# qinzheng93/GeoTransformer

Measured on NVIDIA H100. Metric: point-cloud pairs/sec (3DMatch-shape synth), higher is better.
Workload: dtype f32

## Files before the change

geotransformer_b200/_lib.py:

```python
import ctypes
import os
import threading

import torch

_HERE = os.path.dirname(os.path.abspath(__file__))
LIB_PATH = os.path.join(_HERE, 'libgeob200.so')
_lib = None

c_void_p, c_int64, c_int32, c_float, c_double, c_size_t, c_int = (
    ctypes.c_void_p, ctypes.c_int64, ctypes.c_int32, ctypes.c_float, ctypes.c_double, ctypes.c_size_t, ctypes.c_int)

SIGNATURES = {}


def _sig(name, restype, *argtypes):
    SIGNATURES[name] = (restype, list(argtypes))


P, I64, I32, F, D, SZ = c_void_p, c_int64, c_int32, c_float, c_double, c_size_t
_sig('geob200_last_error', ctypes.c_char_p)
_sig('geob200_launch_count', ctypes.c_uint64)
_sig('geob200_grid_subsample_workspace_bytes', SZ, I64, I64)
_sig('geob200_grid_subsample', c_int, P, I64, P, I64, F, P, P, P, SZ, P)
_sig('geob200_radius_search_workspace_bytes', SZ, I64, I64, I64)
_sig('geob200_radius_search', c_int, P, I64, P, I64, P, P, I64, F, I64, P, P, P, P, SZ, P)

_sig('geob200_neighbor_histogram', c_int, P, I64, I64, I64, I64, P, P)
_sig('geob200_neighbor_histogram_batched', c_int, P, P, P, I64, I64, I64, I64, P, P, P, P)
_sig('geob200_voxel_down_sample_workspace_bytes', SZ, I64, I64)
_sig('geob200_voxel_down_sample', c_int, P, P, I64, P, I64, D, P, P, P, P, SZ, P)
_sig('geob200_estimate_normals_workspace_bytes', SZ, I64, I64)
_sig('geob200_estimate_normals', c_int, P, I64, P, I64, I64, D, P, P, P, P, P, SZ, P)
_sig('geob200_regularize_normals', c_int, P, P, I64, c_int, c_int, P, P)
_sig('geob200_kernel_point_optimize', c_int, P, I64, I64, ctypes.c_uint64, D, P, P, P)
_sig('geob200_kernel_point_instances', c_int, P, I64, P, P, I64, ctypes.c_uint64, P, P)
_sig('geob200_kpconv_workspace_bytes', SZ, I64)
_sig('geob200_kpconv', c_int, P, P, P, P, I64, I64, I64, P, I64, P, P, I64, I64, F, P, P, SZ, P)
_sig('geob200_kpconv_tc_workspace_bytes', SZ, I64, I64, I64)
_sig('geob200_kpconv_tc', c_int, P, P, P, P, I64, I64, I64, P, I64, P, P, I64, I64, F, P, P, SZ, P)
_sig('geob200_set_linear_mode', None, c_int)
_sig('geob200_linear', c_int, P, I64, P, P, P, I64, I64, I64, I64, c_int, P)
_sig('geob200_split_tf32', c_int, P, I64, I64, I64, P, P)
_sig('geob200_linear_batched', c_int, P, I64, I64, P, I64, I64, P, I64, P, I64, I64, I64, I64, I64, I64, c_int, P)
_sig('geob200_group_norm_workspace_bytes', SZ, I64)
_sig('geob200_group_norm', c_int, P, I64, I64, I64, P, P, F, P, c_int, F, P, P, SZ, P)
_sig('geob200_fused_group_norm_workspace_bytes', SZ, I64, I64, I64)
_sig('geob200_linear_group_norm', c_int, P, I64, P, P, I64, I64, I64, I64, P, P, F, P, c_int, F, P, P, P, SZ, P)
_sig('geob200_kpconv_group_norm', c_int, P, P, P, P, I64, I64, I64, P, I64, P, P, I64, I64, F, I64, P, P, F, c_int, F, P, P, P, SZ,
     P, SZ, P)
_sig('geob200_group_norm_batched', c_int, P, I64, I64, I64, P, P, F, P, c_int, F, P, P, SZ, P, I64, P)
_sig('geob200_linear_group_norm_batched', c_int, P, I64, P, P, I64, I64, I64, I64, P, P, F, P, c_int, F, P, P, P, SZ, P, I64, P)
_sig('geob200_maxpool', c_int, P, P, I64, I64, I64, I64, P, P)
_sig('geob200_upsample_concat', c_int, P, P, I64, I64, P, I64, I64, I64, P, P)
_sig('geob200_kpconv_backward_workspace_bytes', SZ, I64, I64, I64, I64, I64)
_sig('geob200_kpconv_backward', c_int, P, P, P, P, I64, I64, I64, P, I64, P, I64, I64, F, P, P, P, P, P, SZ, P)
_sig('geob200_linear_backward_workspace_bytes', SZ, I64, I64, I64, c_int)
_sig('geob200_linear_backward', c_int, P, I64, P, P, I64, I64, I64, P, P, P, P, P, SZ, P)
_sig('geob200_group_norm_backward_batched_workspace_bytes', SZ, I64, I64, I64, I64)
_sig('geob200_group_norm_backward_batched', c_int, P, P, I64, I64, I64, P, F, c_int, F, P, P, P, P, P, P, SZ, P, I64, P)
_sig('geob200_maxpool_backward_batched_workspace_bytes', SZ, I64, I64, I64, I64)
_sig('geob200_maxpool_backward_batched', c_int, P, P, I64, I64, I64, I64, P, I64, P, P, P, P, SZ, P)
_sig('geob200_upsample_concat_backward_workspace_bytes', SZ, I64, I64)
_sig('geob200_upsample_concat_backward', c_int, P, I64, I64, I64, I64, I64, P, P, P, P, SZ, P)
_sig('geob200_point_to_node_partition_batched', c_int, P, P, I64, P, P, I64, P, P, P, P, P, P)
_sig('geob200_gather_rows', c_int, P, I64, I64, P, I64, P, P)
_sig('geob200_knn_partition', c_int, P, I64, P, I64, I64, P, P, P)
_sig('geob200_pairwise_distance', c_int, P, I64, P, I64, I64, c_int, P, P)
_sig('geob200_point_to_node_indices', c_int, P, I64, P, I64, P, P, P)
_sig('geob200_apply_transform', c_int, P, I64, P, P, P)
_sig('geob200_gse_indices_batched', c_int, P, I64, P, F, F, I64, P, P, P)
_sig('geob200_gse_embed_workspace_bytes', SZ, I64, I64)
_sig('geob200_gse_table_bytes', SZ, I64, I64, F, F)
_sig('geob200_gse_table_build', c_int, P, P, P, P, P, I64, I64, F, F, P, SZ, P)
_sig('geob200_gse_embed_table', c_int, P, P, I64, I64, P, SZ, I64, F, F, P, P, P, P, P, P, P)
_sig('geob200_gse_embed_pairs', c_int, P, P, I64, I64, P, P, P, P, P, P, P, P, P, SZ, P)
_sig('geob200_attention_workspace_bytes', SZ, I64, I64, I64)
_sig('geob200_attention', c_int, P, I64, P, I64, P, I64, P, P, P, I64, I64, I64, I64, P, I64, P, SZ, P)
_sig('geob200_set_attention_tma', c_int, c_int)
_sig('geob200_head_bias', c_int, P, I64, P, I64, I64, I64, P, P)
_sig('geob200_add_layernorm', c_int, P, P, P, P, I64, I64, F, P, P)
_sig('geob200_l2_normalize', c_int, P, I64, I64, P, P)
_sig('geob200_add_layernorm_backward_workspace_bytes', SZ, I64, I64)
_sig('geob200_add_layernorm_backward', c_int, P, P, P, I64, I64, F, P, P, P, P, P, SZ, P)
_sig('geob200_l2_normalize_backward', c_int, P, I64, I64, P, P, P)
_sig('geob200_head_project_backward_workspace_bytes', SZ, I64, I64, I64)
_sig('geob200_head_project_backward', c_int, P, I64, P, P, I64, I64, I64, P, P, P, I64, P, P, P, SZ, P)
_sig('geob200_attention_backward_batched_workspace_bytes', SZ, P, I64, I64)
_sig('geob200_attention_backward_batched', c_int, P, P, I64, I64, I64, I64, I64, I64, I64, I64, I64, I64, P, SZ, P)
_sig('geob200_gse_embed_backward_workspace_bytes', SZ, I64, I64)
_sig('geob200_gse_embed_backward', c_int, P, P, I64, I64, I64, P, SZ, I64, F, F, P, P, P, P, P, P, P, P, P, SZ, P)
_sig('geob200_sinkhorn', c_int, P, P, P, P, I64, I64, I64, F, P, P)
_sig('geob200_sinkhorn_backward_workspace_bytes', SZ, I64, I64, I64)
_sig('geob200_sinkhorn_backward', c_int, P, P, P, P, I64, I64, I64, F, P, P, P, P, SZ, P)
_sig('geob200_superpoint_matching_batched_workspace_bytes', SZ, I64, I64, I64)
_sig('geob200_superpoint_matching_batched', c_int, P, P, I64, P, P, I64, P, I64, c_int, P, P, P, P, SZ, P)
_sig('geob200_gather_patches_batched', c_int, P, I64, I64, P, P, P, P, I64, P, P, P, P, P)
_sig('geob200_patch_scores_batched', c_int, P, P, I64, I64, P, P, P, I64, I64, P, P)
_sig('geob200_patch_scores_backward_batched_workspace_bytes', SZ, I64, I64, I64, I64)
_sig('geob200_patch_scores_backward_batched', c_int, P, P, I64, I64, P, P, P, I64, I64, P, P, P, P, SZ, P)
_sig('geob200_lgr_batched_workspace_bytes', SZ, I64, I64, I64, I64)
_sig('geob200_local_global_registration_batched', c_int, P, P, P, P, P, I64, I64, I64, I64, I64, F, c_int, F, I64, I64, P, P, P, P,
     P, P, I64, P, P, P, P, SZ, P)
_sig('geob200_weighted_procrustes', c_int, P, P, P, I64, I64, F, F, P, P)

_sig('geob200_node_correspondences_batched_workspace_bytes', SZ, I64, I64, I64)
_sig('geob200_node_correspondences_batched', c_int, P, P, P, P, P, P, P, P, I64, P, I64, P, F, P, P, P, P, SZ, P)
_sig('geob200_evaluate_counts', c_int, P, P, I64, P, F, P, P, I64, P, P, P, I64, P, F, P, P, P, I64, c_int, F, F, F, P, P)
_sig('geob200_evaluate_batched', c_int, P, P, P, F, P, P, I64, P, P, P, I64, P, F, P, P, I64, P, I64, P, P, c_int, F, F, F, P, I64,
     P)
_sig('geob200_coarse_matching_loss_batched_workspace_bytes', SZ, I64, I64)
_sig('geob200_coarse_matching_loss_batched', c_int, P, P, I64, I64, P, P, P, P, F, F, F, F, F, F, P, I64, P, SZ, P)
_sig('geob200_fine_matching_loss_batched_workspace_bytes', SZ, I64, I64)
_sig('geob200_fine_matching_loss_batched', c_int, P, P, P, P, P, P, I64, I64, I64, P, D, P, P, I64, P, SZ, P)
_sig('geob200_coarse_matching_loss_backward_batched_workspace_bytes', SZ, I64, I64, I64)
_sig('geob200_coarse_matching_loss_backward_batched', c_int, P, P, I64, I64, P, P, P, P, F, F, F, F, F, F, P, I64, P, P, P, P, SZ, P)
_sig('geob200_fine_matching_loss_backward_batched_workspace_bytes', SZ, I64, I64)
_sig('geob200_fine_matching_loss_backward_batched', c_int, P, P, P, P, P, I64, I64, I64, P, D, P, I64, P, P, P, SZ, P)
_sig('geob200_ransac_correspondences_batched_workspace_bytes', SZ, I64, I64)
_sig('geob200_ransac_correspondences_batched', c_int, P, P, I64, I64, P, F, I64, I64, ctypes.c_uint64, I64, P, P, P, P, P, P, P, P, P, P,
     SZ, P)
_sig('geob200_feature_nn_batched_workspace_bytes', SZ, I64, I64, I64)
_sig('geob200_feature_nn_batched', c_int, P, P, I64, I64, I64, I64, P, P, P, P, P, P, P, SZ, P)
_sig('geob200_feature_corr_indices', c_int, P, P, P, P, I64, I64, I32, P, P, P, P, P)
_sig('geob200_ransac_features_batched_workspace_bytes', SZ, I64, I64, I64, I64, I64)
_sig('geob200_ransac_features_batched', c_int, P, P, P, P, I64, I64, I64, I64, P, P, F, I64, I64, I64, ctypes.c_uint64, I64, P, P, P, P, P,
     P, P, P, P, P, P, P, P, P, SZ, P)
_sig('geob200_correspondence_metrics_batched_workspace_bytes', SZ, I64, I64)
_sig('geob200_correspondence_metrics_batched', c_int, P, P, I64, I64, P, P, I64, F, P, I64, P, SZ, P)
_sig('geob200_corr_order_batched', c_int, P, I64, I64, P, I64, P, P)
_sig('geob200_corr_select_batched', c_int, P, P, P, I64, I64, P, P, I64, I64, P, P, P, P, P)
_sig('geob200_sparse_correspondence_eval_batched_workspace_bytes', SZ, I64, I64, I64)
_sig('geob200_sparse_correspondence_eval_batched', c_int, P, P, I64, P, P, I64, P, I64, I64, I64, P, P, SZ, P)
_sig('geob200_registration_error_batched', c_int, P, I64, P, I64, P, P, I64, c_int, D, D, P, P)
_sig('geob200_weighted_procrustes_counts', c_int, P, P, P, I64, I64, P, F, F, P, P)

_sig('geob200_linear_profile_enable', c_int, c_int)
_sig('geob200_set_split_k', c_int, c_int)
_sig('geob200_set_linear_persistent', c_int, c_int)
_sig('geob200_linear_profile_read', I64, I64, P, P)
_sig('geob200_backbone_workspace_bytes', SZ, P, P)
_sig('geob200_backbone_forward_batched', c_int, P, P, P, P, P, P, P, P, P, P, P, P, SZ, P, SZ, P, I64, P, P)
_sig('geob200_cloud_max_count', c_int, P, I64, I64, I64, I64, P, P, P)
_sig('geob200_transformer_batched_workspace_bytes', SZ, I64, P, I64, I64, I64)
_sig('geob200_transformer_forward_batched', c_int, P, I64, I64, I64, P, I64, P, P, P, P, SZ, P)
_sig('geob200_attention_batched_workspace_bytes', SZ, P, I64, I64)
_sig('geob200_attention_batched', c_int, P, I64, I64, I64, I64, I64, I64, I64, P, SZ, P)
_sig('geob200_attention_batched_keeps_probs', c_int, P, I64, I64, I64)
_sig('geob200_superpoint_targets_batched_workspace_bytes', SZ, I64)
_sig('geob200_superpoint_targets_batched', c_int, P, P, P, I64, P, F, I64, ctypes.c_uint64, ctypes.c_uint64, I64, P, P, P, P, SZ, P)
_sig('geob200_nonfinite_check', c_int, P, P, I64, I64, P, P)
_sig('geob200_batch_loss_weights', c_int, P, I64, I64, P, P, P, P, P)
_sig('geob200_kpconv_group_norm_batched', c_int, P, P, P, P, I64, I64, I64, P, I64, P, P, I64, I64, F, I64, P, P, F, c_int, F, P, P, P,
     SZ, P, SZ, P, I64, P)
_sig('geob200_maxpool_batched', c_int, P, P, I64, I64, I64, I64, P, I64, P, P, P)
_sig('geob200_augment_pairs_batched_workspace_bytes', SZ, I64)
_sig('geob200_augment_pairs_batched', c_int, P, P, I64, P, c_int, I64, D, D, D, D, D, ctypes.c_uint64, ctypes.c_uint64, I64, P, P, P, P, P,
     SZ, P)
_sig('geob200_modelnet_pairs_batched_workspace_bytes', SZ, I64)
_sig('geob200_modelnet_pairs_batched', c_int, P, P, I64, I64, D, D, D, D, ctypes.c_uint64, ctypes.c_uint64, I64, P, P, P, P, P, SZ, P)
_sig('geob200_modelnet_benchmark_pairs_batched_workspace_bytes', SZ, I64, I64)
_sig('geob200_modelnet_benchmark_pairs_batched', c_int, P, P, P, I64, I64, D, D, D, D, P, P, P, P, SZ, P)
_sig('geob200_rotated_pairs_batched', c_int, P, c_int, P, P, I64, P, P, P, P, P)
_sig('geob200_modelnet_raw_points_batched_workspace_bytes', SZ, I64)
_sig('geob200_modelnet_raw_points_batched', c_int, P, P, I64, P, P, SZ, P)
_sig('geob200_rpmnet_metrics_batched_workspace_bytes', SZ, I64, I64, I64)
_sig('geob200_rpmnet_metrics_batched', c_int, P, P, P, P, P, P, I64, P, P, P, P, SZ, P)


def lib():
    global _lib
    if _lib is None:
        if not os.path.exists(LIB_PATH):
            raise RuntimeError(
                f'{LIB_PATH} not found: build it with `python -c "import __graft_entry__ as g; g.build()"` '
                '(there is no CPU fallback for the geotransformer_b200 ops)')
        handle = ctypes.CDLL(LIB_PATH)
        for name, (restype, argtypes) in SIGNATURES.items():
            fn = getattr(handle, name)
            fn.restype = restype
            fn.argtypes = argtypes
        _lib = handle
    return _lib


def check(rc, what):
    if rc != 0:
        msg = lib().geob200_last_error().decode(errors='replace')
        raise RuntimeError(f'{what} failed ({rc}): {msg}')


_tls = threading.local()


def stream_ptr():
    p = getattr(_tls, 'stream', None)
    if p is not None:
        return p
    return torch.cuda.current_stream().cuda_stream


class stream_scope:

    def __init__(self, ptr):
        self.ptr = ptr

    def __enter__(self):
        self.prev = getattr(_tls, 'stream', None)
        _tls.stream = self.ptr
        return self

    def __exit__(self, *a):
        _tls.stream = self.prev
        return False


def require_cuda(t, name, dtype=None):
    if not t.is_cuda:
        raise RuntimeError(f'{name} must be a CUDA tensor (geotransformer_b200 has no CPU path)')
    if dtype is not None and t.dtype != dtype:
        raise RuntimeError(f'{name} must be {dtype}, got {t.dtype}')
    if not t.is_contiguous():
        raise RuntimeError(f'{name} must be contiguous')


_WS = {}


def workspace(nbytes, device, tag='default'):
    key = (device.index if device.index is not None else torch.cuda.current_device(), stream_ptr(), tag)
    buf = _WS.get(key)
    if buf is None or buf.numel() < nbytes:
        buf = torch.empty(max(int(nbytes * 1.3), 1 << 20), dtype=torch.uint8, device=device)
        _WS[key] = buf
    return buf


def ptr(t):
    return None if t is None else t.data_ptr()
```

geotransformer_b200/csrc/collate.cu:

```cuda
#include <stdarg.h>
#include <string.h>

#include <mutex>
#include <set>
#include <utility>

#include "common.cuh"
#include "geob200.h"
#include "unordered_map.cuh"

namespace geob200 {

static thread_local char g_err[1024] = "";
static unsigned long long g_launches = 0;
void count_launches(int n) { __atomic_fetch_add(&g_launches, (unsigned long long)n, __ATOMIC_RELAXED); }
void set_error(const char* fmt, ...) {
    va_list ap;
    va_start(ap, fmt);
    vsnprintf(g_err, sizeof(g_err), fmt, ap);
    va_end(ap);
}

int ensure_max_smem(const void* kernel) {
    static std::mutex mu;
    static std::set<std::pair<const void*, int>> done;
    int dev = 0;
    cudaGetDevice(&dev);
    std::lock_guard<std::mutex> lk(mu);
    if (done.count({kernel, dev})) return 0;
    int optin = 0;
    cudaFuncAttributes fa{};
    cudaError_t e = cudaDeviceGetAttribute(&optin, cudaDevAttrMaxSharedMemoryPerBlockOptin, dev);
    if (e == cudaSuccess) e = cudaFuncGetAttributes(&fa, kernel);
    if (e == cudaSuccess) e = cudaFuncSetAttribute(kernel, cudaFuncAttributeMaxDynamicSharedMemorySize, optin - (int)fa.sharedSizeBytes);
    if (e != cudaSuccess) { set_error("ensure_max_smem: %s", cudaGetErrorString(e)); return -1; }
    done.insert({kernel, dev});
    return 0;
}


__global__ void __launch_bounds__(1024) seg_exclusive_scan_kernel(const int* __restrict__ in, int* __restrict__ out,
                                                                  const CloudSeg* __restrict__ segs,
                                                                  int* __restrict__ total) {
    __shared__ int warp_tot[32];
    __shared__ int carry_s;
    const CloudSeg sg = segs[blockIdx.x];
    const int lane = threadIdx.x & 31, warp = threadIdx.x >> 5;
    if (threadIdx.x == 0) carry_s = 0;
    __syncthreads();
    for (int base = 0; base < sg.len; base += 1024) {
        int i = base + threadIdx.x;
        int v = (i < sg.len) ? in[sg.start + i] : 0;
        int x = v;
#pragma unroll
        for (int o = 1; o < 32; o <<= 1) {
            int y = __shfl_up_sync(0xffffffffu, x, o);
            if (lane >= o) x += y;
        }
        if (lane == 31) warp_tot[warp] = x;
        __syncthreads();
        if (warp == 0) {
            int w = warp_tot[lane];
#pragma unroll
            for (int o = 1; o < 32; o <<= 1) {
                int y = __shfl_up_sync(0xffffffffu, w, o);
                if (lane >= o) w += y;
            }
            warp_tot[lane] = w;
        }
        __syncthreads();
        int carry = carry_s;
        int excl = carry + (warp > 0 ? warp_tot[warp - 1] : 0) + (x - v);
        if (i < sg.len) out[sg.start + i] = excl;
        __syncthreads();
        if (threadIdx.x == 1023) carry_s = carry + warp_tot[31];
        __syncthreads();
    }
    if (threadIdx.x == 0 && total != nullptr) total[blockIdx.x] = carry_s;
}


struct GsCloud {
    float ox, oy, oz;
    unsigned long long nx, ny;
};

#define GS_EMPTY 0xFFFFFFFFFFFFFFFFull

__global__ void __launch_bounds__(1024) gs_bounds_kernel(const float* __restrict__ pts, const CloudSeg* __restrict__ segs,
                                                         float voxel, GsCloud* __restrict__ out) {
    const CloudSeg sg = segs[blockIdx.x];
    float mn[3] = {INFINITY, INFINITY, INFINITY}, mx[3] = {-INFINITY, -INFINITY, -INFINITY};
    for (int i = threadIdx.x; i < sg.len; i += blockDim.x) {
        const float* p = pts + 3ll * (sg.start + i);
#pragma unroll
        for (int a = 0; a < 3; ++a) {
            mn[a] = fminf(mn[a], p[a]);
            mx[a] = fmaxf(mx[a], p[a]);
        }
    }
    __shared__ float smn[3][32], smx[3][32];
    const int lane = threadIdx.x & 31, warp = threadIdx.x >> 5;
#pragma unroll
    for (int a = 0; a < 3; ++a) {
#pragma unroll
        for (int o = 16; o > 0; o >>= 1) {
            mn[a] = fminf(mn[a], __shfl_xor_sync(0xffffffffu, mn[a], o));
            mx[a] = fmaxf(mx[a], __shfl_xor_sync(0xffffffffu, mx[a], o));
        }
        if (lane == 0) { smn[a][warp] = mn[a]; smx[a][warp] = mx[a]; }
    }
    __syncthreads();
    if (threadIdx.x == 0) {
        const int nw = blockDim.x >> 5;
        for (int a = 0; a < 3; ++a)
            for (int w = 1; w < nw; ++w) {
                smn[a][0] = fminf(smn[a][0], smn[a][w]);
                smx[a][0] = fmaxf(smx[a][0], smx[a][w]);
            }
        const float inv = (float)(1.0 / (double)voxel);
        GsCloud c;
        c.ox = __fmul_rn(floorf(__fmul_rn(smn[0][0], inv)), voxel);
        c.oy = __fmul_rn(floorf(__fmul_rn(smn[1][0], inv)), voxel);
        c.oz = __fmul_rn(floorf(__fmul_rn(smn[2][0], inv)), voxel);
        c.nx = (unsigned long long)(floorf(__fdiv_rn(__fsub_rn(smx[0][0], c.ox), voxel)) + 1.0f);
        c.ny = (unsigned long long)(floorf(__fdiv_rn(__fsub_rn(smx[1][0], c.oy), voxel)) + 1.0f);
        out[blockIdx.x] = c;
    }
}

__global__ void gs_insert_kernel(const float* __restrict__ pts, const CloudSeg* __restrict__ segs,
                                 const GsCloud* __restrict__ clouds, float voxel,
                                 unsigned long long* __restrict__ tab_key, int* __restrict__ tab_first,
                                 int* __restrict__ pt_slot) {
    const CloudSeg sg = segs[blockIdx.y];
    const int i = blockIdx.x * blockDim.x + threadIdx.x;
    if (i >= sg.len) return;
    const GsCloud c = clouds[blockIdx.y];
    const float* p = pts + 3ll * (sg.start + i);
    unsigned long long ix = (unsigned long long)floorf(__fdiv_rn(__fsub_rn(p[0], c.ox), voxel));
    unsigned long long iy = (unsigned long long)floorf(__fdiv_rn(__fsub_rn(p[1], c.oy), voxel));
    unsigned long long iz = (unsigned long long)floorf(__fdiv_rn(__fsub_rn(p[2], c.oz), voxel));
    unsigned long long key = ix + c.nx * iy + c.nx * c.ny * iz;
    const unsigned tsize = 2u * (unsigned)sg.len;
    const long long tbase = 2ll * sg.start;
    unsigned h = (unsigned)(mix64(key) % tsize);
    while (true) {
        unsigned long long prev = atomicCAS(&tab_key[tbase + h], GS_EMPTY, key);
        if (prev == GS_EMPTY || prev == key) break;
        h = (h + 1 == tsize) ? 0 : h + 1;
    }
    atomicMin(&tab_first[tbase + h], i);
    pt_slot[sg.start + i] = (int)h;
}

__global__ void gs_flag_kernel(const CloudSeg* __restrict__ segs, const int* __restrict__ tab_first,
                               const int* __restrict__ pt_slot, int* __restrict__ flag) {
    const CloudSeg sg = segs[blockIdx.y];
    const int i = blockIdx.x * blockDim.x + threadIdx.x;
    if (i >= sg.len) return;
    flag[sg.start + i] = (tab_first[2ll * sg.start + pt_slot[sg.start + i]] == i) ? 1 : 0;
}

__global__ void gs_offsets_kernel(const int* __restrict__ m, int nb, int* __restrict__ voff, long long* __restrict__ s_lengths) {
    if (threadIdx.x == 0 && blockIdx.x == 0) {
        int acc = 0;
        for (int b = 0; b < nb; ++b) {
            voff[b] = acc;
            acc += m[b];
            s_lengths[b] = m[b];
        }
        voff[nb] = acc;
    }
}

__global__ void gs_voxel_setup_kernel(const float* __restrict__ pts, const CloudSeg* __restrict__ segs,
                                      const GsCloud* __restrict__ clouds, float voxel,
                                      const int* __restrict__ flag, const int* __restrict__ rank,
                                      const int* __restrict__ pt_slot, int* __restrict__ tab_rank,
                                      unsigned long long* __restrict__ vox_key) {
    const CloudSeg sg = segs[blockIdx.y];
    const int i = blockIdx.x * blockDim.x + threadIdx.x;
    if (i >= sg.len) return;
    if (!flag[sg.start + i]) return;
    const GsCloud c = clouds[blockIdx.y];
    const float* p = pts + 3ll * (sg.start + i);
    unsigned long long ix = (unsigned long long)floorf(__fdiv_rn(__fsub_rn(p[0], c.ox), voxel));
    unsigned long long iy = (unsigned long long)floorf(__fdiv_rn(__fsub_rn(p[1], c.oy), voxel));
    unsigned long long iz = (unsigned long long)floorf(__fdiv_rn(__fsub_rn(p[2], c.oz), voxel));
    const int g = rank[sg.start + i];
    tab_rank[2ll * sg.start + pt_slot[sg.start + i]] = g;
    vox_key[sg.start + g] = ix + c.nx * iy + c.nx * c.ny * iz;
}

__global__ void gs_count_kernel(const CloudSeg* __restrict__ segs, const int* __restrict__ tab_rank,
                                const int* __restrict__ pt_slot, int* __restrict__ vox_count) {
    const CloudSeg sg = segs[blockIdx.y];
    const int i = blockIdx.x * blockDim.x + threadIdx.x;
    if (i >= sg.len) return;
    const int g = tab_rank[2ll * sg.start + pt_slot[sg.start + i]];
    atomicAdd(&vox_count[sg.start + g], 1);
}

__global__ void gs_scatter_kernel(const CloudSeg* __restrict__ segs, const int* __restrict__ tab_rank,
                                  const int* __restrict__ pt_slot, const int* __restrict__ vox_off,
                                  int* __restrict__ vox_cursor, int* __restrict__ vox_pts) {
    const CloudSeg sg = segs[blockIdx.y];
    const int i = blockIdx.x * blockDim.x + threadIdx.x;
    if (i >= sg.len) return;
    const int g = tab_rank[2ll * sg.start + pt_slot[sg.start + i]];
    const int pos = atomicAdd(&vox_cursor[sg.start + g], 1);
    vox_pts[sg.start + vox_off[sg.start + g] + pos] = i;
}

__global__ void gs_reduce_kernel(const float* __restrict__ pts, const CloudSeg* __restrict__ segs,
                                 const int* __restrict__ m_per_cloud, const int* __restrict__ vox_off,
                                 const int* __restrict__ vox_count, const int* __restrict__ vox_pts,
                                 float* __restrict__ vox_bary) {
    const CloudSeg sg = segs[blockIdx.y];
    const int g = blockIdx.x * blockDim.x + threadIdx.x;
    if (g >= m_per_cloud[blockIdx.y]) return;
    const int c = vox_count[sg.start + g];
    const int* lst = vox_pts + sg.start + vox_off[sg.start + g];
    float sx = 0.f, sy = 0.f, sz = 0.f;
    int last = -1;
    for (int k = 0; k < c; ++k) {
        int best = 0x7fffffff;
        for (int j = 0; j < c; ++j) {
            int v = lst[j];
            if (v > last && v < best) best = v;
        }
        const float* p = pts + 3ll * (sg.start + best);
        sx = __fadd_rn(sx, p[0]);
        sy = __fadd_rn(sy, p[1]);
        sz = __fadd_rn(sz, p[2]);
        last = best;
    }
    const float w = (float)(1.0 / (double)c);
    float* o = vox_bary + 3ll * (sg.start + g);
    o[0] = __fmul_rn(sx, w);
    o[1] = __fmul_rn(sy, w);
    o[2] = __fmul_rn(sz, w);
}

__global__ void __launch_bounds__(1024) gs_order_kernel(const CloudSeg* __restrict__ segs, const int* __restrict__ m_per_cloud,
                                                        const int* __restrict__ cloud_voff,
                                                        const unsigned long long* __restrict__ vox_key,
                                                        const float* __restrict__ vox_bary,
                                                        int* __restrict__ cur_g, int* __restrict__ nxt_g,
                                                        int* __restrict__ A_g, int* __restrict__ lnk_g,
                                                        int* __restrict__ bucket_scratch,
                                                        float* __restrict__ s_points) {
    const CloudSeg sg = segs[blockIdx.x];
    const int m = m_per_cloud[blockIdx.x];
    int* act = bucket_scratch + (3ll * sg.start + 64ll * blockIdx.x) * 3;
    const long long bcap = 3ll * sg.len + 64;
    const int* order = unordered_map_order(m, vox_key + sg.start, cur_g + sg.start, nxt_g + sg.start, A_g + sg.start,
                                           lnk_g + sg.start, act, act + bcap, act + 2 * bcap);
    float* out = s_points + 3ll * cloud_voff[blockIdx.x];
    for (int q = threadIdx.x; q < m; q += blockDim.x) {
        const float* bsrc = vox_bary + 3ll * (sg.start + order[q]);
        out[3 * q + 0] = bsrc[0];
        out[3 * q + 1] = bsrc[1];
        out[3 * q + 2] = bsrc[2];
    }
}

static int upload_segs(const int64_t* lengths_h, int64_t batch, CloudSeg* d_segs, int64_t* total, int* max_len,
                       cudaStream_t st) {
    CloudSeg tmp[64];
    CloudSeg* h = tmp;
    CloudSeg* heap = nullptr;
    if (batch > 64) { heap = (CloudSeg*)malloc(sizeof(CloudSeg) * batch); h = heap; }
    int64_t acc = 0;
    int mx = 0;
    for (int64_t b = 0; b < batch; ++b) {
        h[b].start = (int)acc;
        h[b].len = (int)lengths_h[b];
        acc += lengths_h[b];
        if ((int)lengths_h[b] > mx) mx = (int)lengths_h[b];
    }
    cudaError_t e = cudaMemcpyAsync(d_segs, h, sizeof(CloudSeg) * batch, cudaMemcpyHostToDevice, st);
    if (heap) { cudaStreamSynchronize(st); free(heap); }
    *total = acc;
    *max_len = mx;
    if (e != cudaSuccess) { set_error("upload_segs: %s", cudaGetErrorString(e)); return -1; }
    return 0;
}


struct RsCloud {
    float ox, oy, oz;
    float cell;
    int cx, cy, cz;
    int cell_base;
};

__global__ void __launch_bounds__(1024) rs_bounds_kernel(const float* __restrict__ pts, const CloudSeg* __restrict__ segs,
                                                         float radius, RsCloud* __restrict__ out, CloudSeg* __restrict__ cell_segs,
                                                         int* __restrict__ max_count) {
    if (blockIdx.x == 0 && threadIdx.x == 0) *max_count = 0;
    const CloudSeg sg = segs[blockIdx.x];
    float mn[3] = {INFINITY, INFINITY, INFINITY}, mx[3] = {-INFINITY, -INFINITY, -INFINITY};
    for (int i = threadIdx.x; i < sg.len; i += blockDim.x) {
        const float* p = pts + 3ll * (sg.start + i);
#pragma unroll
        for (int a = 0; a < 3; ++a) { mn[a] = fminf(mn[a], p[a]); mx[a] = fmaxf(mx[a], p[a]); }
    }
    __shared__ float smn[3][32], smx[3][32];
    const int lane = threadIdx.x & 31, warp = threadIdx.x >> 5;
#pragma unroll
    for (int a = 0; a < 3; ++a) {
#pragma unroll
        for (int o = 16; o > 0; o >>= 1) {
            mn[a] = fminf(mn[a], __shfl_xor_sync(0xffffffffu, mn[a], o));
            mx[a] = fmaxf(mx[a], __shfl_xor_sync(0xffffffffu, mx[a], o));
        }
        if (lane == 0) { smn[a][warp] = mn[a]; smx[a][warp] = mx[a]; }
    }
    __syncthreads();
    if (threadIdx.x == 0) {
        const int nw = blockDim.x >> 5;
        for (int a = 0; a < 3; ++a)
            for (int w = 1; w < nw; ++w) { smn[a][0] = fminf(smn[a][0], smn[a][w]); smx[a][0] = fmaxf(smx[a][0], smx[a][w]); }
        RsCloud c;
        c.ox = smn[0][0]; c.oy = smn[1][0]; c.oz = smn[2][0];
        const long long budget = 2ll * sg.len + 1024;
        float cell = radius * 1.001f;
        long long cx, cy, cz;
        while (true) {
            cx = (long long)floorf((smx[0][0] - c.ox) / cell) + 1;
            cy = (long long)floorf((smx[1][0] - c.oy) / cell) + 1;
            cz = (long long)floorf((smx[2][0] - c.oz) / cell) + 1;
            if (cx <= 1024 && cy <= 1024 && cz <= 1024 && cx * cy * cz <= budget) break;
            cell *= 1.25f;
        }
        c.cell = cell; c.cx = (int)cx; c.cy = (int)cy; c.cz = (int)cz;
        c.cell_base = 2 * sg.start + 1025 * blockIdx.x;
        out[blockIdx.x] = c;
        cell_segs[blockIdx.x].start = c.cell_base;
        cell_segs[blockIdx.x].len = c.cx * c.cy * c.cz + 1;
    }
}

__device__ __forceinline__ int rs_cell_of(const RsCloud& c, float x, float y, float z) {
    int ix = (int)floorf((x - c.ox) / c.cell), iy = (int)floorf((y - c.oy) / c.cell), iz = (int)floorf((z - c.oz) / c.cell);
    ix = min(max(ix, 0), c.cx - 1); iy = min(max(iy, 0), c.cy - 1); iz = min(max(iz, 0), c.cz - 1);
    return (iz * c.cy + iy) * c.cx + ix;
}

__global__ void rs_count_kernel(const float* __restrict__ pts, const CloudSeg* __restrict__ segs,
                                const RsCloud* __restrict__ clouds, int* __restrict__ cell_cnt, int* __restrict__ pt_cell) {
    const CloudSeg sg = segs[blockIdx.y];
    const int i = blockIdx.x * blockDim.x + threadIdx.x;
    if (i >= sg.len) return;
    const RsCloud c = clouds[blockIdx.y];
    const float* p = pts + 3ll * (sg.start + i);
    const int cell = rs_cell_of(c, p[0], p[1], p[2]);
    pt_cell[sg.start + i] = cell;
    atomicAdd(&cell_cnt[c.cell_base + cell], 1);
}

__global__ void rs_scatter_kernel(const float* __restrict__ pts, const CloudSeg* __restrict__ segs,
                                  const RsCloud* __restrict__ clouds, const int* __restrict__ cell_start,
                                  int* __restrict__ cell_cursor, const int* __restrict__ pt_cell,
                                  float4* __restrict__ sorted) {
    const CloudSeg sg = segs[blockIdx.y];
    const int i = blockIdx.x * blockDim.x + threadIdx.x;
    if (i >= sg.len) return;
    const RsCloud c = clouds[blockIdx.y];
    const int cell = pt_cell[sg.start + i];
    const int pos = atomicAdd(&cell_cursor[c.cell_base + cell], 1);
    const float* p = pts + 3ll * (sg.start + i);
    sorted[sg.start + cell_start[c.cell_base + cell] + pos] = make_float4(p[0], p[1], p[2], __int_as_float(i));
}

struct RsSegs {
    int start, len;
};
__global__ void rs_cellsegs_kernel(const RsCloud* __restrict__ clouds, int nb, CloudSeg* __restrict__ cell_segs) {
    int b = blockIdx.x * blockDim.x + threadIdx.x;
    if (b >= nb) return;
    const RsCloud c = clouds[b];
    cell_segs[b].start = c.cell_base;
    cell_segs[b].len = c.cx * c.cy * c.cz + 1;
}

template <int KPL>
__device__ __forceinline__ void warp_bitonic_sort(unsigned long long (&key)[KPL], int lane) {
#pragma unroll
    for (int k = 2; k <= 32 * KPL; k <<= 1) {
#pragma unroll
        for (int j = k >> 1; j > 0; j >>= 1) {
            if (j >= 32) {
                const int rj = j >> 5;
#pragma unroll
                for (int r = 0; r < KPL; ++r) {
                    if ((r & rj) == 0) {
                        const bool up = (((r * 32 + lane) & k) == 0);
                        const unsigned long long a = key[r], b = key[r | rj];
                        const bool swap = (a > b) == up;
                        key[r] = swap ? b : a;
                        key[r | rj] = swap ? a : b;
                    }
                }
            } else {
#pragma unroll
                for (int r = 0; r < KPL; ++r) {
                    const unsigned long long a = key[r];
                    const unsigned long long b = __shfl_xor_sync(0xffffffffu, a, j);
                    const bool up = (((r * 32 + lane) & k) == 0);
                    const bool lower = (lane & j) == 0;
                    const bool take_min = (up == lower);
                    key[r] = take_min ? (a < b ? a : b) : (a > b ? a : b);
                }
            }
        }
    }
}

template <int KPL>
__device__ __forceinline__ void rs_sort_and_store(const unsigned long long* buf, int count, int lane, long long* orow, int width,
                                                  long long start, long long sentinel) {
    unsigned long long key[KPL];
#pragma unroll
    for (int r = 0; r < KPL; ++r) key[r] = (r * 32 + lane < count) ? buf[r * 32 + lane] : 0xFFFFFFFFFFFFFFFFull;
    warp_bitonic_sort<KPL>(key, lane);
#pragma unroll
    for (int r = 0; r < KPL; ++r) {
        const int e = r * 32 + lane;
        if (e < width) orow[e] = (e < count) ? (long long)(unsigned)(key[r] & 0xFFFFFFFFull) + start : sentinel;
    }
    for (int e = 32 * KPL + lane; e < width; e += 32) orow[e] = sentinel;
}

template <int CAP>
__device__ __forceinline__ void rs_query_body(unsigned long long* buf, int lane, int b, int qi,
                                              const float* __restrict__ q_pts, const CloudSeg* __restrict__ q_segs,
                                              const CloudSeg* __restrict__ s_segs, const RsCloud* __restrict__ clouds,
                                              const int* __restrict__ cell_start, const float4* __restrict__ sorted,
                                              float radius, int width, long long sentinel, long long* __restrict__ out,
                                              int* __restrict__ counts, int* __restrict__ max_count,
                                              int* __restrict__ overflow_list, int* __restrict__ overflow_n) {
    const CloudSeg qs = q_segs[b];
    const CloudSeg ss = s_segs[b];
    const RsCloud c = clouds[b];
    const long long row = (long long)qs.start + qi;
    const float qx = q_pts[3 * row], qy = q_pts[3 * row + 1], qz = q_pts[3 * row + 2];
    const float r2 = __fmul_rn(radius, radius);
    const float lim = 2.0e6f;
    const int ix = (int)fminf(fmaxf(floorf((qx - c.ox) / c.cell), -lim), lim);
    const int iy = (int)fminf(fmaxf(floorf((qy - c.oy) / c.cell), -lim), lim);
    const int iz = (int)fminf(fmaxf(floorf((qz - c.oz) / c.cell), -lim), lim);
    int count = 0;
    const int x0 = max(ix - 1, 0), x1 = min(ix + 1, c.cx - 1);
    if (x0 <= x1) {
        for (int dz = -1; dz <= 1; ++dz) {
            const int z = iz + dz;
            if (z < 0 || z >= c.cz) continue;
            for (int dy = -1; dy <= 1; ++dy) {
                const int y = iy + dy;
                if (y < 0 || y >= c.cy) continue;
                const int rowcell = c.cell_base + (z * c.cy + y) * c.cx;
                const int beg = cell_start[rowcell + x0], end = cell_start[rowcell + x1 + 1];
                const int end_pad = beg + ((end - beg + 31) / 32) * 32;
                for (int k = beg + lane; k < end_pad; k += 32) {
                    bool hit = false;
                    unsigned long long kv = 0;
                    if (k < end) {
                        const float4 s = sorted[ss.start + k];
                        const float ex = __fsub_rn(qx, s.x), ey = __fsub_rn(qy, s.y), ez = __fsub_rn(qz, s.z);
                        float d = __fmul_rn(ex, ex);
                        d = __fadd_rn(d, __fmul_rn(ey, ey));
                        d = __fadd_rn(d, __fmul_rn(ez, ez));
                        hit = d < r2;
                        kv = ((unsigned long long)__float_as_uint(d) << 32) | (unsigned)__float_as_int(s.w);
                    }
                    const unsigned msk = __ballot_sync(0xffffffffu, hit);
                    if (hit) {
                        const int pos = count + __popc(msk & ((1u << lane) - 1u));
                        if (pos < CAP) buf[pos] = kv;
                    }
                    count += __popc(msk);
                }
            }
        }
    }
    if (count > CAP) {
        if (lane == 0) {
            if (overflow_list != nullptr) overflow_list[atomicAdd(overflow_n, 1)] = (int)row;
            else atomicExch(max_count, -1 << 30);
        }
        return;
    }
    if (lane == 0) {
        if (counts != nullptr) counts[row] = count;
        atomicMax(max_count, count);
    }
    if (out == nullptr || width <= 0) return;
    __syncwarp();
    long long* orow = out + row * (long long)width;
    if (count <= 32) rs_sort_and_store<1>(buf, count, lane, orow, width, ss.start, sentinel);
    else if (count <= 64) rs_sort_and_store<2>(buf, count, lane, orow, width, ss.start, sentinel);
    else if (count <= 128) rs_sort_and_store<4>(buf, count, lane, orow, width, ss.start, sentinel);
    else if (count <= 256) rs_sort_and_store<8>(buf, count, lane, orow, width, ss.start, sentinel);
    else {
        int n2 = 1;
        while (n2 < count) n2 <<= 1;
        for (int k = count + lane; k < n2; k += 32) buf[k] = 0xFFFFFFFFFFFFFFFFull;
        __syncwarp();
        for (int k = 2; k <= n2; k <<= 1) {
            for (int j = k >> 1; j > 0; j >>= 1) {
                for (int t = lane; t < n2; t += 32) {
                    const int p = t ^ j;
                    if (p > t) {
                        const unsigned long long a = buf[t], bb = buf[p];
                        const bool up = ((t & k) == 0);
                        if ((a > bb) == up) { buf[t] = bb; buf[p] = a; }
                    }
                }
                __syncwarp();
            }
        }
        for (int k = lane; k < width; k += 32)
            orow[k] = (k < count) ? (long long)(unsigned)(buf[k] & 0xFFFFFFFFull) + ss.start : sentinel;
    }
}

template <int CAP>
__global__ void rs_query_kernel(const float* __restrict__ q_pts, const CloudSeg* __restrict__ q_segs,
                                const CloudSeg* __restrict__ s_segs, const RsCloud* __restrict__ clouds,
                                const int* __restrict__ cell_start, const float4* __restrict__ sorted, float radius,
                                int width, long long sentinel, long long* __restrict__ out, int* __restrict__ counts,
                                int* __restrict__ max_count, int* __restrict__ overflow_list, int* __restrict__ overflow_n) {
    extern __shared__ unsigned long long smem_keys[];
    const int warps_per_block = blockDim.x >> 5;
    const int lane = threadIdx.x & 31, warp = threadIdx.x >> 5;
    const int b = blockIdx.y;
    const int qi = blockIdx.x * warps_per_block + warp;
    if (qi >= q_segs[b].len) return;
    rs_query_body<CAP>(smem_keys + (size_t)warp * CAP, lane, b, qi, q_pts, q_segs, s_segs, clouds, cell_start, sorted,
                       radius, width, sentinel, out, counts, max_count, overflow_list, overflow_n);
}

template <int CAP>
__global__ void rs_redo_kernel(const float* __restrict__ q_pts, const CloudSeg* __restrict__ q_segs,
                               const CloudSeg* __restrict__ s_segs, const RsCloud* __restrict__ clouds,
                               const int* __restrict__ cell_start, const float4* __restrict__ sorted, float radius,
                               int width, long long sentinel, long long* __restrict__ out, int* __restrict__ counts,
                               int* __restrict__ max_count, const int* __restrict__ redo_list,
                               const int* __restrict__ redo_n, int nbatch) {
    extern __shared__ unsigned long long smem_keys[];
    const int n = *redo_n;
    for (int w = blockIdx.x; w < n; w += gridDim.x) {
        const int row = redo_list[w];
        int b = 0;
        while (b + 1 < nbatch && row >= q_segs[b + 1].start) ++b;
        rs_query_body<CAP>(smem_keys, threadIdx.x, b, row - q_segs[b].start, q_pts, q_segs, s_segs, clouds, cell_start,
                           sorted, radius, width, sentinel, out, counts, max_count, nullptr, nullptr);
        __syncwarp();
    }
}

__global__ void __launch_bounds__(256) neighbor_histogram_kernel(const long long* __restrict__ nbr, long long rows, int width,
                                                                 long long n_support, int hist_n, int* __restrict__ hist) {
    const long long r = (long long)blockIdx.x * blockDim.x + threadIdx.x;
    if (r >= rows) return;
    int c = 0;
    for (int j = 0; j < width; ++j) c += nbr[r * width + j] < n_support ? 1 : 0;
    if (c < hist_n) atomicAdd(&hist[c], 1);
}

struct HistStages {
    const long long* nbr[GEOB200_MAX_STAGES];
    long long rows[GEOB200_MAX_STAGES];
    int width[GEOB200_MAX_STAGES];
    int cloud_start[GEOB200_MAX_STAGES][2 * GEOB200_HIST_MAX_PAIRS + 1];
};

__global__ void __launch_bounds__(256) neighbor_histogram_batched_kernel(HistStages st, int num_stages, int batch, int hist_n,
                                                                         int* __restrict__ hists) {
    const int s = blockIdx.y;
    const long long r = (long long)blockIdx.x * blockDim.x + threadIdx.x;
    if (r >= st.rows[s]) return;
    const int w = st.width[s];
    const long long* row = st.nbr[s] + r * w;
    int c = 0;
    for (int j = 0; j < w; ++j) c += row[j] < st.rows[s] ? 1 : 0;
    if (c >= hist_n) return;
    int cloud = 0;
    while (cloud + 1 < 2 * batch && r >= st.cloud_start[s][cloud + 1]) ++cloud;
    atomicAdd(&hists[((size_t)(cloud % batch) * num_stages + s) * hist_n + c], 1);
}

__global__ void __launch_bounds__(256) neighbor_histogram_stop_kernel(const int* __restrict__ hists, int num_stages, int batch,
                                                                      int hist_n, long long threshold, int* __restrict__ totals,
                                                                      int* __restrict__ stop) {
    __shared__ long long row_sum[GEOB200_HIST_MAX_PAIRS * GEOB200_MAX_STAGES];
    __shared__ long long base[GEOB200_MAX_STAGES];
    __shared__ int last;
    const int t = threadIdx.x;
    for (int i = t; i < batch * num_stages; i += blockDim.x) {
        long long v = 0;
        for (int h = 0; h < hist_n; ++h) v += hists[(size_t)i * hist_n + h];
        row_sum[i] = v;
    }
    for (int s = t; s < num_stages; s += blockDim.x) {
        long long v = 0;
        for (int h = 0; h < hist_n; ++h) v += totals[(size_t)s * hist_n + h];
        base[s] = v;
    }
    __syncthreads();
    if (t == 0) {
        int found = -1;
        for (int p = 0; p < batch && found < 0; ++p) {
            bool all = true;
            for (int s = 0; s < num_stages; ++s) {
                base[s] += row_sum[p * num_stages + s];
                all = all && base[s] > threshold;
            }
            if (all) found = p;
        }
        *stop = found;
        last = found >= 0 ? found : batch - 1;
    }
    __syncthreads();
    for (int i = t; i < num_stages * hist_n; i += blockDim.x) {
        int v = totals[i];
        for (int p = 0; p <= last; ++p) v += hists[(size_t)p * num_stages * hist_n + i];
        totals[i] = v;
    }
}

}

using namespace geob200;

extern "C" {

const char* geob200_last_error(void) { return g_err; }
uint64_t geob200_launch_count(void) { return g_launches; }

size_t geob200_grid_subsample_workspace_bytes(int64_t n_points, int64_t batch) {
    size_t n = (size_t)n_points, b = (size_t)batch;
    size_t bytes = 0;
    bytes += align_up(sizeof(CloudSeg) * b, 256) + align_up(sizeof(GsCloud) * b, 256);
    bytes += align_up(8 * 2 * n, 256) + align_up(4 * 2 * n, 256) * 2;
    bytes += align_up(4 * n, 256) * 11;
    bytes += align_up(8 * n, 256);
    bytes += align_up(12 * n, 256);
    bytes += align_up(4 * 3 * (3 * n + 64 * b), 256);
    bytes += align_up(4 * (b + 1), 256) * 2;
    return bytes + 4096;
}

int geob200_grid_subsample(const float* points, int64_t n_points, const int64_t* lengths_h, int64_t batch, float voxel,
                           float* s_points, int64_t* s_lengths, void* workspace, size_t workspace_bytes, void* stream) {
    cudaStream_t st = (cudaStream_t)stream;
    GEOB_REQUIRE(batch > 0 && n_points > 0, "grid_subsample: empty input (n=%lld, batch=%lld)", (long long)n_points, (long long)batch);
    GEOB_REQUIRE(voxel > 0.f, "grid_subsample: voxel size must be positive");
    GEOB_REQUIRE(n_points < (1ll << 30), "grid_subsample: too many points");
    for (int64_t b = 0; b < batch; ++b)
        GEOB_REQUIRE(lengths_h[b] > 0, "grid_subsample: cloud %lld is empty (the reference reads points[0])", (long long)b);
    GEOB_REQUIRE(workspace_bytes >= geob200_grid_subsample_workspace_bytes(n_points, batch), "grid_subsample: workspace too small");
    Arena ar(workspace, workspace_bytes);
    const size_t n = (size_t)n_points;
    CloudSeg* segs = ar.take<CloudSeg>(batch);
    GsCloud* clouds = ar.take<GsCloud>(batch);
    unsigned long long* tab_key = ar.take<unsigned long long>(2 * n);
    int* tab_first = ar.take<int>(2 * n);
    int* tab_rank = ar.take<int>(2 * n);
    int* pt_slot = ar.take<int>(n);
    int* flag = ar.take<int>(n);
    int* rank = ar.take<int>(n);
    int* vox_count = ar.take<int>(2 * n);
    int* vox_cursor = vox_count + n;
    int* vox_off = ar.take<int>(n);
    int* vox_pts = ar.take<int>(n);
    int* cur = ar.take<int>(n);
    int* nxt = ar.take<int>(n);
    int* A = ar.take<int>(n);
    int* lnk = ar.take<int>(n);
    unsigned long long* vox_key = ar.take<unsigned long long>(n);
    float* vox_bary = ar.take<float>(3 * n);
    int* bucket_scratch = ar.take<int>(3 * (3 * n + 64 * (size_t)batch));
    int* m_per_cloud = ar.take<int>(batch + 1);
    int* voff = ar.take<int>(batch + 1);
    GEOB_REQUIRE(ar.ok(), "grid_subsample: workspace accounting error");

    int64_t total = 0;
    int max_len = 0;
    if (upload_segs(lengths_h, batch, segs, &total, &max_len, st)) return -1;
    GEOB_REQUIRE(total == n_points, "grid_subsample: sum(lengths)=%lld != n_points=%lld", (long long)total, (long long)n_points);

    GEOB_CHECK_CUDA(cudaMemsetAsync(tab_key, 0xFF, 8 * 2 * n, st));
    GEOB_CHECK_CUDA(cudaMemsetAsync(tab_first, 0x7F, 4 * 2 * n, st));
    GEOB_CHECK_CUDA(cudaMemsetAsync(vox_count, 0, 4 * 2 * n, st));

    const dim3 pgrid((max_len + 255) / 256, (unsigned)batch);
    gs_bounds_kernel<<<(unsigned)batch, 1024, 0, st>>>(points, segs, voxel, clouds);
    gs_insert_kernel<<<pgrid, 256, 0, st>>>(points, segs, clouds, voxel, tab_key, tab_first, pt_slot);
    gs_flag_kernel<<<pgrid, 256, 0, st>>>(segs, tab_first, pt_slot, flag);
    seg_exclusive_scan_kernel<<<(unsigned)batch, 1024, 0, st>>>(flag, rank, segs, m_per_cloud);
    gs_offsets_kernel<<<1, 32, 0, st>>>(m_per_cloud, (int)batch, voff, (long long*)s_lengths);
    gs_voxel_setup_kernel<<<pgrid, 256, 0, st>>>(points, segs, clouds, voxel, flag, rank, pt_slot, tab_rank, vox_key);
    gs_count_kernel<<<pgrid, 256, 0, st>>>(segs, tab_rank, pt_slot, vox_count);
    seg_exclusive_scan_kernel<<<(unsigned)batch, 1024, 0, st>>>(vox_count, vox_off, segs, nullptr);
    gs_scatter_kernel<<<pgrid, 256, 0, st>>>(segs, tab_rank, pt_slot, vox_off, vox_cursor, vox_pts);
    gs_reduce_kernel<<<pgrid, 256, 0, st>>>(points, segs, m_per_cloud, vox_off, vox_count, vox_pts, vox_bary);
    gs_order_kernel<<<(unsigned)batch, 1024, 0, st>>>(segs, m_per_cloud, voff, vox_key, vox_bary, cur, nxt, A, lnk,
                                                     bucket_scratch, s_points);
    GEOB_CHECK_LAUNCH();
    count_launches(11);
    return 0;
}

size_t geob200_radius_search_workspace_bytes(int64_t n_query, int64_t n_support, int64_t batch) {
    size_t ns = (size_t)n_support, nq = (size_t)n_query, b = (size_t)batch;
    size_t cells = 2 * ns + 1025 * b + 64;
    size_t bytes = 0;
    bytes += align_up(sizeof(CloudSeg) * b, 256) * 3 + align_up(sizeof(RsCloud) * b, 256);
    bytes += align_up(4 * cells, 256) * 3 + 1024;
    bytes += align_up(4 * ns, 256);
    bytes += align_up(16 * ns, 256);
    bytes += align_up(4 * nq, 256);
    bytes += 1024;
    return bytes + 4096;
}

int geob200_radius_search(const float* q_points, int64_t n_query, const float* s_points, int64_t n_support,
                          const int64_t* q_lengths_h, const int64_t* s_lengths_h, int64_t batch, float radius,
                          int64_t width, int64_t* out, int32_t* counts, int32_t* max_count, void* workspace,
                          size_t workspace_bytes, void* stream) {
    cudaStream_t st = (cudaStream_t)stream;
    GEOB_REQUIRE(batch > 0 && n_query > 0 && n_support > 0, "radius_search: empty input");
    GEOB_REQUIRE(radius > 0.f, "radius_search: radius must be positive");
    GEOB_REQUIRE(max_count != nullptr, "radius_search: max_count output is required");
    GEOB_REQUIRE(n_query < (1ll << 30) && n_support < (1ll << 30), "radius_search: too many points");
    GEOB_REQUIRE(workspace_bytes >= geob200_radius_search_workspace_bytes(n_query, n_support, batch), "radius_search: workspace too small");
    for (int64_t b = 0; b < batch; ++b)
        GEOB_REQUIRE(q_lengths_h[b] >= 0 && s_lengths_h[b] > 0, "radius_search: cloud %lld has no support points", (long long)b);
    Arena ar(workspace, workspace_bytes);
    const size_t ns = (size_t)n_support;
    const size_t cells = 2 * ns + 1025 * (size_t)batch + 64;
    CloudSeg* q_segs = ar.take<CloudSeg>(batch);
    CloudSeg* s_segs = ar.take<CloudSeg>(batch);
    CloudSeg* cell_segs = ar.take<CloudSeg>(batch);
    RsCloud* clouds = ar.take<RsCloud>(batch);
    int* zero_block = ar.take<int>(2 * cells + 64);
    int* cell_cnt = zero_block;
    int* cell_cursor = zero_block + cells;
    int* overflow_n = zero_block + 2 * cells;
    int* cell_start = ar.take<int>(cells);
    int* pt_cell = ar.take<int>(ns);
    float4* sorted = ar.take<float4>(ns);
    int* overflow_list = ar.take<int>((size_t)n_query);
    GEOB_REQUIRE(ar.ok(), "radius_search: workspace accounting error");

    int64_t tq = 0, ts = 0;
    int max_q = 0, max_s = 0;
    if (upload_segs(q_lengths_h, batch, q_segs, &tq, &max_q, st)) return -1;
    if (upload_segs(s_lengths_h, batch, s_segs, &ts, &max_s, st)) return -1;
    GEOB_REQUIRE(tq == n_query && ts == n_support, "radius_search: lengths do not sum to the row counts");

    GEOB_CHECK_CUDA(cudaMemsetAsync(zero_block, 0, 4 * (2 * cells + 64), st));

    const dim3 sgrid((max_s + 255) / 256, (unsigned)batch);
    rs_bounds_kernel<<<(unsigned)batch, 1024, 0, st>>>(s_points, s_segs, radius, clouds, cell_segs, max_count);
    rs_count_kernel<<<sgrid, 256, 0, st>>>(s_points, s_segs, clouds, cell_cnt, pt_cell);
    seg_exclusive_scan_kernel<<<(unsigned)batch, 1024, 0, st>>>(cell_cnt, cell_start, cell_segs, nullptr);
    rs_scatter_kernel<<<sgrid, 256, 0, st>>>(s_points, s_segs, clouds, cell_start, cell_cursor, pt_cell, sorted);
    if (max_q > 0) {
        constexpr int CAP = 256, WARPS = 4;
        const dim3 qgrid((max_q + WARPS - 1) / WARPS, (unsigned)batch);
        rs_query_kernel<CAP><<<qgrid, WARPS * 32, WARPS * CAP * 8, st>>>(
            q_points, q_segs, s_segs, clouds, cell_start, sorted, radius, (int)width, (long long)n_support,
            (long long*)out, counts, max_count, overflow_list, overflow_n);
        constexpr int CAP2 = 16384;
        if (ensure_max_smem((const void*)rs_redo_kernel<CAP2>)) return -1;
        rs_redo_kernel<CAP2><<<num_sms(), 32, CAP2 * 8, st>>>(
            q_points, q_segs, s_segs, clouds, cell_start, sorted, radius, (int)width, (long long)n_support,
            (long long*)out, counts, max_count, overflow_list, overflow_n, (int)batch);
        count_launches(2);
    }
    GEOB_CHECK_LAUNCH();
    count_launches(4);
    return 0;
}

int geob200_neighbor_histogram(const int64_t* neighbors, int64_t n_rows, int64_t width, int64_t n_support, int64_t hist_n,
                               int32_t* hist, void* stream) {
    GEOB_REQUIRE(n_rows > 0 && width > 0 && hist_n > 0, "neighbor_histogram: empty input");
    neighbor_histogram_kernel<<<(unsigned)((n_rows + 255) / 256), 256, 0, (cudaStream_t)stream>>>(
        (const long long*)neighbors, (long long)n_rows, (int)width, (long long)n_support, (int)hist_n, hist);
    GEOB_CHECK_LAUNCH();
    count_launches(1);
    return 0;
}

int geob200_neighbor_histogram_batched(const int64_t* const* neighbors, const int64_t* widths, const int64_t* cloud_rows,
                                       int64_t num_stages, int64_t batch, int64_t hist_n, int64_t sample_threshold, int32_t* hists,
                                       int32_t* totals, int32_t* stop, void* stream) {
    GEOB_REQUIRE(num_stages >= 1 && num_stages <= GEOB200_MAX_STAGES, "neighbor_histogram_batched: num_stages must be in 1..%d",
                 GEOB200_MAX_STAGES);
    GEOB_REQUIRE(batch >= 1 && batch <= GEOB200_HIST_MAX_PAIRS, "neighbor_histogram_batched: batch must be in 1..%d",
                 GEOB200_HIST_MAX_PAIRS);
    GEOB_REQUIRE(hist_n >= 1 && hist_n <= (1 << 20), "neighbor_histogram_batched: hist_n must be in 1..2^20");
    GEOB_REQUIRE(neighbors != nullptr && widths != nullptr && cloud_rows != nullptr && hists != nullptr && totals != nullptr &&
                 stop != nullptr, "neighbor_histogram_batched: null pointer");
    HistStages st;
    long long max_rows = 0;
    for (int s = 0; s < (int)num_stages; ++s) {
        GEOB_REQUIRE(neighbors[s] != nullptr && widths[s] >= 1 && widths[s] <= (1 << 20),
                     "neighbor_histogram_batched: stage %d has no table or a bad width", s);
        long long row = 0;
        for (int c = 0; c < 2 * (int)batch; ++c) {
            GEOB_REQUIRE(cloud_rows[s * 2 * batch + c] >= 1, "neighbor_histogram_batched: stage %d cloud %d is empty", s, c);
            st.cloud_start[s][c] = (int)row;
            row += cloud_rows[s * 2 * batch + c];
            GEOB_REQUIRE(row < (1LL << 31), "neighbor_histogram_batched: stage %d has 2^31 rows or more", s);
        }
        st.cloud_start[s][2 * batch] = (int)row;
        st.nbr[s] = (const long long*)neighbors[s];
        st.rows[s] = row;
        st.width[s] = (int)widths[s];
        max_rows = row > max_rows ? row : max_rows;
    }
    cudaStream_t cs = (cudaStream_t)stream;
    GEOB_CHECK_CUDA(cudaMemsetAsync(hists, 0, sizeof(int32_t) * (size_t)batch * num_stages * hist_n, cs));
    neighbor_histogram_batched_kernel<<<dim3((unsigned)((max_rows + 255) / 256), (unsigned)num_stages), 256, 0, cs>>>(
        st, (int)num_stages, (int)batch, (int)hist_n, hists);
    neighbor_histogram_stop_kernel<<<1, 256, 0, cs>>>(hists, (int)num_stages, (int)batch, (int)hist_n, (long long)sample_threshold,
                                                      totals, stop);
    GEOB_CHECK_LAUNCH();
    count_launches(2);
    return 0;
}

}
```

geotransformer_b200/ext.py:

```python

import torch

from . import _lib as L


def _prep(points, lengths, pname, lname):
    if points.dtype != torch.float32:
        raise RuntimeError(f'{pname} must be a float tensor')
    if lengths.dtype != torch.int64:
        raise RuntimeError(f'{lname} must be an long tensor')
    if not points.is_contiguous():
        raise RuntimeError(f'{pname} must be contiguous')
    if not lengths.is_contiguous():
        raise RuntimeError(f'{lname} must be contiguous')
    was_cpu = not points.is_cuda
    if was_cpu:
        points = points.cuda()
    lengths_h = lengths.cpu() if lengths.is_cuda else lengths
    return points, lengths_h, was_cpu


def grid_subsampling(points, lengths, voxel_size):
    dev_lengths = lengths.device
    points, lengths_h, was_cpu = _prep(points, lengths, 'points', 'lengths')
    n, b = points.shape[0], lengths_h.shape[0]
    lib = L.lib()
    ws_bytes = lib.geob200_grid_subsample_workspace_bytes(n, b)
    ws = L.workspace(ws_bytes, points.device)
    s_points = torch.empty((n, 3), dtype=torch.float32, device=points.device)
    s_lengths = torch.empty((b,), dtype=torch.int64, device=points.device)
    L.check(lib.geob200_grid_subsample(points.data_ptr(), n, lengths_h.data_ptr(), b, float(voxel_size),
                                       s_points.data_ptr(), s_lengths.data_ptr(), ws.data_ptr(), ws.numel(),
                                       L.stream_ptr()), 'grid_subsampling')
    s_lengths_h = s_lengths.cpu()
    total = int(s_lengths_h.sum())
    s_points = s_points[:total].clone()
    if was_cpu:
        return [s_points.cpu(), s_lengths_h]
    return [s_points, s_lengths if dev_lengths.type == 'cuda' else s_lengths_h]


def _radius_call(q_points, s_points, ql_h, sl_h, radius, width, out, counts, max_count):
    lib = L.lib()
    nq, ns, b = q_points.shape[0], s_points.shape[0], ql_h.shape[0]
    ws_bytes = lib.geob200_radius_search_workspace_bytes(nq, ns, b)
    ws = L.workspace(ws_bytes, q_points.device)
    L.check(lib.geob200_radius_search(q_points.data_ptr(), nq, s_points.data_ptr(), ns, ql_h.data_ptr(),
                                      sl_h.data_ptr(), b, float(radius), int(width), L.ptr(out), L.ptr(counts),
                                      max_count.data_ptr(), ws.data_ptr(), ws.numel(), L.stream_ptr()),
            'radius_neighbors')


def radius_neighbors(q_points, s_points, q_lengths, s_lengths, radius, neighbor_limit=0):
    q_points, ql_h, was_cpu = _prep(q_points, q_lengths, 'q_points', 'q_lengths')
    s_points, sl_h, _ = _prep(s_points, s_lengths, 's_points', 's_lengths')
    nq = q_points.shape[0]
    dev = q_points.device
    max_count = torch.zeros((1,), dtype=torch.int32, device=dev)
    if neighbor_limit > 0:
        out = torch.empty((nq, neighbor_limit), dtype=torch.int64, device=dev)
        _radius_call(q_points, s_points, ql_h, sl_h, radius, neighbor_limit, out, None, max_count)
        mc = int(max_count.item())
        if mc < 0:
            raise RuntimeError('radius_neighbors: more than 16384 neighbours for one query')
        if mc < neighbor_limit:
            out = out[:, :mc].contiguous()
    else:
        _radius_call(q_points, s_points, ql_h, sl_h, radius, 0, None, None, max_count)
        mc = int(max_count.item())
        if mc < 0:
            raise RuntimeError('radius_neighbors: more than 16384 neighbours for one query')
        out = torch.empty((nq, mc), dtype=torch.int64, device=dev)
        if mc > 0:
            _radius_call(q_points, s_points, ql_h, sl_h, radius, mc, out, None, max_count)
    return out.cpu() if was_cpu else out


def radius_neighbors_deferred(q_points, s_points, q_lengths, s_lengths, radius, neighbor_limit):
    q_points, ql_h, _ = _prep(q_points, q_lengths, 'q_points', 'q_lengths')
    s_points, sl_h, _ = _prep(s_points, s_lengths, 's_points', 's_lengths')
    dev = q_points.device
    max_count = torch.empty((1,), dtype=torch.int32, device=dev)
    out = torch.empty((q_points.shape[0], neighbor_limit), dtype=torch.int64, device=dev)
    _radius_call(q_points, s_points, ql_h, sl_h, radius, neighbor_limit, out, None, max_count)
    return out, max_count
```

geotransformer_b200/modules/ops/__init__.py:

```python
import torch

from ... import ext as _ext
from ... import functional as GF


def grid_subsample(points, lengths, voxel_size):
    s_points, s_lengths = _ext.grid_subsampling(points, lengths, voxel_size)
    return s_points, s_lengths


def radius_search(q_points, s_points, q_lengths, s_lengths, radius, neighbor_limit):
    return _ext.radius_neighbors(q_points, s_points, q_lengths, s_lengths, radius, neighbor_limit=max(int(neighbor_limit), 0))


def radius_search_deferred(q_points, s_points, q_lengths, s_lengths, radius, neighbor_limit):
    return _ext.radius_neighbors_deferred(q_points, s_points, q_lengths, s_lengths, radius, int(neighbor_limit))


def point_to_node_partition(points, nodes, point_limit, return_count=False):
    return GF.point_to_node_partition(points, nodes, point_limit, return_count)


def knn_partition(points, nodes, k, return_distance=False):
    return GF.knn_partition(points, nodes, k, return_distance)


def get_point_to_node_indices(points, nodes, return_counts=False):
    return GF.point_to_node_indices(points, nodes, return_counts)


def ball_query_partition(points, nodes, radius, point_limit, return_count=False):
    node_knn_distances, node_knn_indices = GF.knn_partition(points, nodes, point_limit, return_distance=True)
    node_knn_masks = torch.lt(node_knn_distances, radius)
    node_knn_indices = torch.where(node_knn_masks, node_knn_indices, torch.full_like(node_knn_indices, points.shape[0]))
    if return_count:
        return node_knn_indices, node_knn_masks, node_knn_masks.sum(1)
    return node_knn_indices, node_knn_masks


def pairwise_distance(x, y, normalized=False, channel_first=False):
    return GF.pairwise_distance(x, y, normalized, channel_first)


def index_select(data, index, dim):
    if dim == 0 and data.is_cuda and data.dtype == torch.float32 and data.ndim == 2 and data.is_contiguous():
        return GF.gather_rows(data, index.contiguous())
    out = data.index_select(dim, index.reshape(-1))
    if index.ndim > 1:
        out = out.view(*data.shape[:dim], *index.shape, *data.shape[dim:][1:])
    return out


def apply_transform(points, transform):
    if transform.ndim == 2:
        return GF.apply_transform(points, transform.contiguous())
    return torch.stack([GF.apply_transform(p, t.contiguous()) for p, t in zip(points, transform)])
```

geotransformer_b200/utils/data.py:

```python
import ctypes

import numpy as np
import torch

from ..modules.ops import grid_subsample, radius_search_deferred


def precompute_data_stack_mode(points, lengths, num_stages, voxel_size, radius, neighbor_limits):
    assert num_stages == len(neighbor_limits)
    points_list, lengths_list, lengths_host = [], [], []
    for i in range(num_stages):
        if i > 0:
            points, lengths = grid_subsample(points, lengths_host[-1], voxel_size=voxel_size)
        lengths_h = lengths.cpu() if lengths.is_cuda else lengths
        points_list.append(points)
        lengths_host.append(lengths_h)
        lengths_list.append(lengths_h.to(points.device))
        voxel_size *= 2

    pending = []
    for i in range(num_stages):
        cur_points, cur_lengths = points_list[i], lengths_host[i]
        pending.append(('n', radius_search_deferred(cur_points, cur_points, cur_lengths, cur_lengths, radius, neighbor_limits[i])))
        if i < num_stages - 1:
            sub_points, sub_lengths = points_list[i + 1], lengths_host[i + 1]
            pending.append(('s', radius_search_deferred(sub_points, cur_points, sub_lengths, cur_lengths, radius, neighbor_limits[i])))
            pending.append(('u', radius_search_deferred(cur_points, sub_points, cur_lengths, sub_lengths, radius * 2,
                                                        neighbor_limits[i + 1])))
        radius *= 2
    counts = torch.stack([p[1][1] for p in pending]).cpu().flatten().tolist()
    neighbors_list, subsampling_list, upsampling_list = [], [], []
    for (kind, (table, _)), mc in zip(pending, counts):
        if mc < 0:
            raise RuntimeError('radius_search: more than 16384 neighbours for one query')
        if mc < table.shape[1]:
            table = table[:, :mc].contiguous()
        {'n': neighbors_list, 's': subsampling_list, 'u': upsampling_list}[kind].append(table)
    return {'points': points_list, 'lengths': lengths_list, 'lengths_host': [l.tolist() for l in lengths_host],
            'neighbors': neighbors_list, 'subsampling': subsampling_list, 'upsampling': upsampling_list}


def _stack_to_device(tensors, device):
    if all(t.is_cuda for t in tensors):
        return tensors[0] if len(tensors) == 1 else torch.cat(tensors, dim=0)
    total = sum(int(t.shape[0]) for t in tensors)
    out = torch.empty((total,) + tuple(tensors[0].shape[1:]), dtype=tensors[0].dtype, device=device)
    row = 0
    for t in tensors:
        out[row:row + t.shape[0]].copy_(t, non_blocking=True)
        row += t.shape[0]
    return out


def registration_collate_fn_stack_mode(data_dicts, num_stages, voxel_size, search_radius, neighbor_limits,
                                       precompute_data=True, device='cuda'):
    batch_size = len(data_dicts)
    collated = {}
    for d in data_dicts:
        for key, value in d.items():
            if isinstance(value, np.ndarray):
                value = torch.from_numpy(value)
            collated.setdefault(key, []).append(value)
    feats_list = collated.pop('ref_feats') + collated.pop('src_feats')
    points_list = collated.pop('ref_points') + collated.pop('src_points')
    lengths = torch.LongTensor([p.shape[0] for p in points_list])
    if batch_size == 1:
        for key, value in collated.items():
            collated[key] = value[0]
    def _dev(v):
        if isinstance(v, torch.Tensor):
            return v.to(device, non_blocking=True)
        if isinstance(v, list) and v and all(isinstance(x, torch.Tensor) for x in v):
            return [x.to(device, non_blocking=True) for x in v]
        return v
    collated = {k: _dev(v) for k, v in collated.items()}
    points, feats = _stack_to_device(points_list, device), _stack_to_device(feats_list, device)
    collated['features'] = feats
    if precompute_data:
        collated.update(precompute_data_stack_mode(points, lengths, num_stages, voxel_size, search_radius, neighbor_limits))
    else:
        collated['points'] = points
        collated['lengths'] = lengths
    collated['batch_size'] = batch_size
    return collated


def calibrate_neighbors_stack_mode(dataset, collate_fn, num_stages, voxel_size, search_radius, keep_ratio=0.8, sample_threshold=2000):
    from .. import _lib as L
    hist_n = int(np.ceil(4 / 3 * np.pi * (search_radius / voxel_size + 1) ** 3))
    max_neighbor_limits = [hist_n] * num_stages
    hists = None
    lib = L.lib()
    for i in range(len(dataset)):
        data_dict = collate_fn([dataset[i]], num_stages, voxel_size, search_radius, max_neighbor_limits, precompute_data=True)
        if hists is None:
            hists = torch.zeros((num_stages, hist_n), dtype=torch.int32, device=data_dict['neighbors'][0].device)
        for s, neighbors in enumerate(data_dict['neighbors']):
            L.check(lib.geob200_neighbor_histogram(neighbors.data_ptr(), neighbors.shape[0], neighbors.shape[1], neighbors.shape[0],
                                                   hist_n, hists[s].data_ptr(), L.stream_ptr()), 'neighbor_histogram')
        if int(hists.sum(dim=1).min().item()) > sample_threshold:
            break
    neighbor_hists = hists.cpu().numpy()
    cum_sum = np.cumsum(neighbor_hists.T, axis=0)
    neighbor_limits = np.sum(cum_sum < (keep_ratio * cum_sum[hist_n - 1, :]), axis=0)
    return neighbor_limits


CALIBRATION_ITERATION = (1 << 64) - 1
HIST_MAX_PAIRS = 32


def calibrate_neighbors_augmented(pairs, cfg, seed, keep_ratio=0.8, sample_threshold=2000, chunk=16, device=None):
    from .. import _lib as L
    from ..augment import augment_stacked
    if not 1 <= chunk <= HIST_MAX_PAIRS:
        raise ValueError(f'chunk must be in 1..{HIST_MAX_PAIRS}')
    device = torch.device('cuda', torch.cuda.current_device()) if device is None else torch.device(device)
    b = cfg.backbone
    S, voxel_size, radius = b.num_stages, b.init_voxel_size, b.init_radius
    hist_n = int(np.ceil(4 / 3 * np.pi * (radius / voxel_size + 1) ** 3))
    totals = torch.zeros((S, hist_n), dtype=torch.int32, device=device)
    hists = torch.empty((chunk, S, hist_n), dtype=torch.int32, device=device)
    stop = torch.empty((1,), dtype=torch.int32, device=device)
    lib = L.lib()
    n, used = len(pairs), len(pairs)
    with torch.cuda.device(device):
        for base in range(0, n, chunk):
            group = [pairs[i] for i in range(base, min(n, base + chunk))]
            B = len(group)
            points, lengths, _, _, _ = augment_stacked(group, cfg, seed, CALIBRATION_ITERATION, device, pair_base=base)
            data = precompute_data_stack_mode(points, torch.LongTensor(lengths), S, voxel_size, radius, [hist_n] * S)
            tables = data['neighbors']
            ptrs = (ctypes.c_void_p * S)(*[t.data_ptr() for t in tables])
            widths = np.array([t.shape[1] for t in tables], dtype=np.int64)
            rows = np.array(data['lengths_host'], dtype=np.int64).reshape(S, 2 * B)
            L.check(lib.geob200_neighbor_histogram_batched(ptrs, widths.ctypes.data, rows.ctypes.data, S, B, hist_n, sample_threshold,
                                                           hists.data_ptr(), totals.data_ptr(), stop.data_ptr(), L.stream_ptr()),
                    'neighbor_histogram_batched')
            p = int(stop.item())
            if p >= 0:
                used = base + p + 1
                break
    cum_sum = np.cumsum(totals.cpu().numpy().T, axis=0)
    return np.sum(cum_sum < (keep_ratio * cum_sum[hist_n - 1, :]), axis=0), used
```

include/geob200.h:

```cpp
#ifndef GEOB200_H
#define GEOB200_H

#include <stddef.h>
#include <stdint.h>

#ifdef __cplusplus
extern "C" {
#endif

const char* geob200_last_error(void);
uint64_t geob200_launch_count(void);


size_t geob200_grid_subsample_workspace_bytes(int64_t n_points, int64_t batch);
int geob200_grid_subsample(const float* points, int64_t n_points, const int64_t* lengths_h, int64_t batch, float voxel,
                           float* s_points, int64_t* s_lengths, void* workspace, size_t workspace_bytes, void* stream);

size_t geob200_radius_search_workspace_bytes(int64_t n_query, int64_t n_support, int64_t batch);
int geob200_radius_search(const float* q_points, int64_t n_query, const float* s_points, int64_t n_support,
                          const int64_t* q_lengths_h, const int64_t* s_lengths_h, int64_t batch, float radius,
                          int64_t width, int64_t* out, int32_t* counts, int32_t* max_count, void* workspace,
                          size_t workspace_bytes, void* stream);

int geob200_neighbor_histogram(const int64_t* neighbors, int64_t n_rows, int64_t width, int64_t n_support, int64_t hist_n,
                               int32_t* hist, void* stream);

#define GEOB200_HIST_MAX_PAIRS 32
int geob200_neighbor_histogram_batched(const int64_t* const* neighbors, const int64_t* widths, const int64_t* cloud_rows,
                                       int64_t num_stages, int64_t batch, int64_t hist_n, int64_t sample_threshold, int32_t* hists,
                                       int32_t* totals, int32_t* stop, void* stream);


#define GEOB200_VOXEL_MAX_CLOUDS 64
#define GEOB200_VOXEL_NONFINITE 1
#define GEOB200_VOXEL_TOO_SMALL 2
#define GEOB200_VOXEL_AXIS_LIMIT 3
size_t geob200_voxel_down_sample_workspace_bytes(int64_t n_points, int64_t batch);
int geob200_voxel_down_sample(const double* points, const double* normals, int64_t n_points, const int64_t* lengths_h, int64_t batch,
                              double voxel, double* out_points, double* out_normals, int64_t* out_lengths, void* workspace,
                              size_t workspace_bytes, void* stream);


#define GEOB200_NORMALS_MAX_CLOUDS 64
#define GEOB200_NORMALS_MAX_KNN 64
#define GEOB200_NORMALS_NONFINITE 1
size_t geob200_estimate_normals_workspace_bytes(int64_t n_points, int64_t batch);
int geob200_estimate_normals(const double* points, int64_t n_points, const int64_t* lengths_h, int64_t batch, int64_t knn, double radius,
                             double* out_normals, int32_t* out_neighbors, double* out_covariance, int64_t* out_status, void* workspace,
                             size_t workspace_bytes, void* stream);
int geob200_regularize_normals(const void* points, const void* normals, int64_t n, int fp64, int positive, double* out, void* stream);


#define GEOB200_KP_MAX_POINTS 30
int geob200_kernel_point_optimize(const double* init, int64_t num_kernels, int64_t num_points, uint64_t seed, double ratio,
                                  double* points, int32_t* info, void* stream);

int geob200_kernel_point_instances(const double* disposition, int64_t num_points, const double* radii, const int64_t* layer_ids,
                                   int64_t num_layers, uint64_t seed, float* out, void* stream);


size_t geob200_kpconv_workspace_bytes(int64_t n_support);
int geob200_kpconv(const float* s_feats, const float* q_points, const float* s_points, const int64_t* neighbors,
                   int64_t n_query, int64_t n_support, int64_t n_neighbors, const float* kernel_points, int64_t n_kernel,
                   const float* weights, const float* bias, int64_t c_in, int64_t c_out, float sigma, float* out,
                   void* workspace, size_t workspace_bytes, void* stream);

size_t geob200_kpconv_tc_workspace_bytes(int64_t n_query, int64_t n_support, int64_t c_in);
int geob200_kpconv_tc(const float* s_feats, const float* q_points, const float* s_points, const int64_t* neighbors, int64_t n_query,
                      int64_t n_support, int64_t n_neighbors, const float* kernel_points, int64_t n_kernel, const float* weights_t,
                      const float* bias, int64_t c_in, int64_t c_out, float sigma, float* out, void* workspace, size_t workspace_bytes,
                      void* stream);

int geob200_split_tf32(const float* w, int64_t ld, int64_t n, int64_t k, float* out, void* stream);

void geob200_set_linear_mode(int mode);
int geob200_linear(const float* x, int64_t ldx, const float* weight, const float* bias, float* y, int64_t ldy, int64_t m,
                   int64_t n, int64_t k, int relu, void* stream);
int geob200_linear_batched(const float* x, int64_t ldx, int64_t stride_x, const float* weight, int64_t ldw, int64_t stride_w,
                           const float* bias, int64_t stride_b, float* y, int64_t ldy, int64_t stride_y, int64_t m, int64_t n,
                           int64_t k, int64_t batch, int relu, void* stream);

size_t geob200_group_norm_workspace_bytes(int64_t groups);
int geob200_group_norm(const float* x, int64_t n_rows, int64_t channels, int64_t groups, const float* gamma,
                       const float* beta, float eps, const float* residual, int leaky, float slope, float* y,
                       void* workspace, size_t workspace_bytes, void* stream);

size_t geob200_fused_group_norm_workspace_bytes(int64_t n_rows, int64_t channels, int64_t groups);
int geob200_linear_group_norm(const float* x, int64_t ldx, const float* weight, const float* bias, int64_t m, int64_t n, int64_t k,
                              int64_t groups, const float* gamma, const float* beta, float eps, const float* residual, int leaky,
                              float slope, float* pre_norm, float* y, void* workspace, size_t workspace_bytes, void* stream);
int geob200_kpconv_group_norm(const float* s_feats, const float* q_points, const float* s_points, const int64_t* neighbors,
                              int64_t n_query, int64_t n_support, int64_t n_neighbors, const float* kernel_points, int64_t n_kernel,
                              const float* weights_t, const float* bias, int64_t c_in, int64_t c_out, float sigma, int64_t groups,
                              const float* gamma, const float* beta, float eps, int leaky, float slope, float* pre_norm, float* y,
                              void* gn_workspace, size_t gn_workspace_bytes, void* workspace, size_t workspace_bytes, void* stream);

int geob200_group_norm_batched(const float* x, int64_t n_rows, int64_t channels, int64_t groups, const float* gamma, const float* beta,
                               float eps, const float* residual, int leaky, float slope, float* y, void* workspace, size_t workspace_bytes,
                               void* stream, int64_t n_pairs, const int64_t* cloud_rows_h);
int geob200_linear_group_norm_batched(const float* x, int64_t ldx, const float* weight, const float* bias, int64_t m, int64_t n, int64_t k,
                                      int64_t groups, const float* gamma, const float* beta, float eps, const float* residual, int leaky,
                                      float slope, float* pre_norm, float* y, void* workspace, size_t workspace_bytes, void* stream,
                                      int64_t n_pairs, const int64_t* cloud_rows_h);
int geob200_kpconv_group_norm_batched(const float* s_feats, const float* q_points, const float* s_points, const int64_t* neighbors,
                                      int64_t n_query, int64_t n_support, int64_t n_neighbors, const float* kernel_points, int64_t n_kernel,
                                      const float* weights_t, const float* bias, int64_t c_in, int64_t c_out, float sigma, int64_t groups,
                                      const float* gamma, const float* beta, float eps, int leaky, float slope, float* pre_norm, float* y,
                                      void* gn_workspace, size_t gn_workspace_bytes, void* workspace, size_t workspace_bytes, void* stream,
                                      int64_t n_pairs, const int64_t* cloud_rows_h);

int geob200_maxpool(const float* x, const int64_t* neighbors, int64_t n_query, int64_t n_support, int64_t n_neighbors,
                    int64_t channels, float* y, void* stream);
int geob200_maxpool_batched(const float* x, const int64_t* neighbors, int64_t n_query, int64_t n_support, int64_t n_neighbors,
                            int64_t channels, const int32_t* cloud_max, int64_t n_pairs, const int64_t* cloud_rows_h, float* y,
                            void* stream);

int geob200_cloud_max_count(const int64_t* neighbors, int64_t n_query, int64_t n_support, int64_t n_neighbors, int64_t n_pairs,
                            const int64_t* cloud_rows_h, int32_t* cloud_max, void* stream);

int geob200_upsample_concat(const float* x, const int64_t* up_indices, int64_t up_stride, int64_t n_support,
                            const float* skip, int64_t n_query, int64_t c1, int64_t c2, float* y, void* stream);


size_t geob200_kpconv_backward_workspace_bytes(int64_t n_query, int64_t n_support, int64_t n_neighbors, int64_t c_in, int64_t c_out);
int geob200_kpconv_backward(const float* s_feats, const float* q_points, const float* s_points, const int64_t* neighbors, int64_t n_query,
                            int64_t n_support, int64_t n_neighbors, const float* kernel_points, int64_t n_kernel, const float* weights,
                            int64_t c_in, int64_t c_out, float sigma, const float* grad_out, float* grad_feats, float* grad_weights,
                            float* grad_bias, void* workspace, size_t workspace_bytes, void* stream);

size_t geob200_linear_backward_workspace_bytes(int64_t m, int64_t n, int64_t k, int relu);
int geob200_linear_backward(const float* x, int64_t ldx, const float* weight_t, const float* relu_y, int64_t m, int64_t n, int64_t k,
                            const float* grad_y, float* grad_x, float* grad_weight, float* grad_bias, void* workspace, size_t workspace_bytes,
                            void* stream);

size_t geob200_group_norm_backward_batched_workspace_bytes(int64_t n_rows, int64_t channels, int64_t groups, int64_t n_pairs);
int geob200_group_norm_backward_batched(const float* x, const float* y, int64_t n_rows, int64_t channels, int64_t groups, const float* gamma,
                                        float eps, int leaky, float slope, const float* grad_y, float* grad_x, float* grad_gamma,
                                        float* grad_beta, float* grad_residual, void* workspace, size_t workspace_bytes, void* stream,
                                        int64_t n_pairs, const int64_t* cloud_rows_h);

size_t geob200_maxpool_backward_batched_workspace_bytes(int64_t n_query, int64_t n_support, int64_t n_neighbors, int64_t channels);
int geob200_maxpool_backward_batched(const float* x, const int64_t* neighbors, int64_t n_query, int64_t n_support, int64_t n_neighbors,
                                     int64_t channels, const int32_t* cloud_max, int64_t n_pairs, const int64_t* cloud_rows_h,
                                     const float* grad_y, float* grad_x, void* workspace, size_t workspace_bytes, void* stream);

size_t geob200_upsample_concat_backward_workspace_bytes(int64_t n_query, int64_t n_support);
int geob200_upsample_concat_backward(const int64_t* up_indices, int64_t up_stride, int64_t n_query, int64_t n_support, int64_t c1, int64_t c2,
                                     const float* grad_y, float* grad_x, float* grad_skip, void* workspace, size_t workspace_bytes,
                                     void* stream);


int geob200_point_to_node_partition_batched(const float* points, const float* nodes, int64_t n_clouds, const int64_t* cloud_points,
                                            const int64_t* cloud_nodes, int64_t point_limit, int64_t* point_to_node, uint8_t* node_masks,
                                            int32_t* node_sizes, int64_t* node_knn_indices, uint8_t* node_knn_masks, void* stream);

int geob200_knn_partition(const float* points, int64_t n_points, const float* nodes, int64_t n_nodes, int64_t k,
                          int64_t* knn_indices, float* knn_sq_distances, void* stream);
int geob200_pairwise_distance(const float* x, int64_t n, const float* y, int64_t m, int64_t channels, int normalized, float* out,
                              void* stream);
int geob200_point_to_node_indices(const float* points, int64_t n_points, const float* nodes, int64_t n_nodes, int64_t* indices,
                                  int32_t* node_sizes, void* stream);
int geob200_apply_transform(const float* points, int64_t n_points, const float* transform, float* out, void* stream);

int geob200_gather_rows(const float* table, int64_t n_rows, int64_t channels, const int64_t* indices, int64_t n_indices,
                        float* out, void* stream);


int geob200_gse_indices_batched(const float* points, int64_t n_clouds, const int64_t* cloud_rows_h, float sigma_d, float factor_a,
                                int64_t angle_k, float* d_indices, float* a_indices, void* stream);

size_t geob200_gse_embed_workspace_bytes(int64_t n, int64_t channels);
int geob200_gse_embed_pairs(const float* d_indices, const float* a_indices, int64_t n_rows, int64_t channels, const float* div_term,
                            const float* wd_t, const float* wa_t, const float* wd, const float* wa, const float* bd, const float* ba,
                            float* embeddings, void* workspace, size_t workspace_bytes, void* stream);

size_t geob200_gse_table_bytes(int64_t channels, int64_t inv_step, float d_max, float a_max);
int geob200_gse_table_build(const float* div_term, const float* wd_t, const float* wa_t, const float* bd, const float* ba,
                            int64_t channels, int64_t inv_step, float d_max, float a_max, void* table, size_t table_bytes,
                            void* stream);
int geob200_gse_embed_table(const float* d_indices, const float* a_indices, int64_t n_rows, int64_t channels, const void* table,
                            size_t table_bytes, int64_t inv_step, float d_max, float a_max, const float* div_term, const float* wd,
                            const float* wa, const float* bd, const float* ba, float* embeddings, void* stream);

size_t geob200_attention_workspace_bytes(int64_t n_query, int64_t n_key, int64_t heads);
int geob200_attention(const float* q, int64_t ldq, const float* k, int64_t ldk, const float* v, int64_t ldv, const float* qp,
                      const float* qb, const float* embed, int64_t n_query, int64_t n_key, int64_t channels, int64_t heads,
                      float* out, int64_t ldo, void* workspace, size_t workspace_bytes, void* stream);
#define GEOB200_ATT_MAX_ITEMS 32
typedef struct { const float* q; const float* k; const float* v; const float* qp; const float* qb; const float* embed; float* out;
                 int64_t n_query, n_key; } geob200_att_item_t;
size_t geob200_attention_batched_workspace_bytes(const geob200_att_item_t* items_h, int64_t n_items, int64_t heads);
int geob200_attention_batched(const geob200_att_item_t* items_h, int64_t n_items, int64_t ldq, int64_t ldk, int64_t ldv, int64_t ldo,
                              int64_t channels, int64_t heads, void* workspace, size_t workspace_bytes, void* stream);
int geob200_attention_batched_keeps_probs(const geob200_att_item_t* items_h, int64_t n_items, int64_t channels, int64_t heads);
int geob200_set_attention_tma(int on);
int geob200_head_bias(const float* q, int64_t ldq, const float* bias_p, int64_t n, int64_t channels, int64_t heads, float* qb,
                      void* stream);
int geob200_add_layernorm(const float* a, const float* b, const float* gamma, const float* beta, int64_t n, int64_t channels,
                          float eps, float* y, void* stream);
int geob200_l2_normalize(const float* x, int64_t n, int64_t channels, float* y, void* stream);


size_t geob200_add_layernorm_backward_workspace_bytes(int64_t n, int64_t channels);
int geob200_add_layernorm_backward(const float* a, const float* b, const float* gamma, int64_t n, int64_t channels, float eps,
                                   const float* grad_y, float* grad_x, float* grad_gamma, float* grad_beta, void* workspace,
                                   size_t workspace_bytes, void* stream);
int geob200_l2_normalize_backward(const float* x, int64_t n, int64_t channels, const float* grad_y, float* grad_x, void* stream);
size_t geob200_head_project_backward_workspace_bytes(int64_t n, int64_t channels, int64_t heads);
int geob200_head_project_backward(const float* q, int64_t ldq, const float* wp, const float* bp, int64_t n, int64_t channels, int64_t heads,
                                  const float* grad_qp, const float* grad_qb, float* grad_q, int64_t ldgq, float* grad_wp, float* grad_bp,
                                  void* workspace, size_t workspace_bytes, void* stream);
typedef struct { const float* probs; const float* grad_out; float* grad_q; float* grad_k; float* grad_v; float* grad_qp; float* grad_qb;
                 float* grad_embed; } geob200_att_grad_item_t;
size_t geob200_attention_backward_batched_workspace_bytes(const geob200_att_item_t* items_h, int64_t n_items, int64_t heads);
int geob200_attention_backward_batched(const geob200_att_item_t* items_h, const geob200_att_grad_item_t* grads_h, int64_t n_items,
                                       int64_t ldq, int64_t ldk, int64_t ldv, int64_t ldo, int64_t ldgq, int64_t ldgk, int64_t ldgv,
                                       int64_t channels, int64_t heads, void* workspace, size_t workspace_bytes, void* stream);
size_t geob200_gse_embed_backward_workspace_bytes(int64_t n_rows, int64_t channels);
int geob200_gse_embed_backward(const float* d_indices, const float* a_indices, int64_t n_rows, int64_t angle_k, int64_t channels,
                               const void* table, size_t table_bytes, int64_t inv_step, float d_max, float a_max, const float* div_term,
                               const float* wa, const float* ba, const float* grad_embed, float* grad_wd, float* grad_bd, float* grad_wa,
                               float* grad_ba, void* workspace, size_t workspace_bytes, void* stream);


size_t geob200_superpoint_matching_batched_workspace_bytes(int64_t n_rows, int64_t n_products, int64_t n_pairs);
int geob200_superpoint_matching_batched(const float* ref_feats, const float* src_feats, int64_t channels, const uint8_t* ref_masks,
                                        const uint8_t* src_masks, int64_t n_pairs, const int64_t* cloud_nodes, int64_t num_correspondences,
                                        int dual, int64_t* corr_indices, float* corr_scores, int32_t* num_out, void* workspace,
                                        size_t workspace_bytes, void* stream);

int geob200_gather_patches_batched(const int64_t* corr_indices, int64_t n_corr, int64_t n_clouds, const int64_t* cloud_nodes,
                                   const int64_t* cloud_points, const int64_t* node_knn_indices, const uint8_t* node_knn_masks, int64_t k,
                                   const float* points, int64_t* out_indices, uint8_t* out_masks, float* out_points, void* stream);

int geob200_patch_scores_batched(const float* ref_feats, const float* src_feats, int64_t channels, int64_t n_pairs, const int64_t* cloud_points,
                                 const int64_t* ref_knn_indices, const int64_t* src_knn_indices, int64_t n_patches, int64_t k,
                                 float* scores, void* stream);

size_t geob200_patch_scores_backward_batched_workspace_bytes(int64_t n_rows, int64_t n_patches_total, int64_t k, int64_t channels);
int geob200_patch_scores_backward_batched(const float* ref_feats, const float* src_feats, int64_t channels, int64_t n_pairs,
                                          const int64_t* cloud_points, const int64_t* ref_knn_indices, const int64_t* src_knn_indices,
                                          int64_t n_patches, int64_t k, const float* grad_scores, float* grad_ref_feats,
                                          float* grad_src_feats, void* workspace, size_t workspace_bytes, void* stream);

int geob200_sinkhorn(const float* scores, const uint8_t* row_masks, const uint8_t* col_masks, const float* alpha,
                     int64_t n_patches, int64_t k, int64_t num_iterations, float inf, float* out, void* stream);

size_t geob200_sinkhorn_backward_workspace_bytes(int64_t n_patches, int64_t k, int64_t num_iterations);
int geob200_sinkhorn_backward(const float* scores, const uint8_t* row_masks, const uint8_t* col_masks, const float* alpha, int64_t n_patches,
                              int64_t k, int64_t num_iterations, float inf, const float* grad_out, float* grad_scores, float* grad_alpha,
                              void* workspace, size_t workspace_bytes, void* stream);


size_t geob200_lgr_batched_workspace_bytes(int64_t n_pairs, int64_t n_patches, int64_t k, int64_t topk);
int geob200_local_global_registration_batched(const float* ref_knn_points, const float* src_knn_points, const uint8_t* ref_knn_masks,
                                              const uint8_t* src_knn_masks, const float* log_scores, int64_t n_pairs, int64_t n_patches,
                                              int64_t k, int64_t score_ld, int64_t topk, float acceptance_radius, int mutual,
                                              float confidence_threshold, int64_t correspondence_threshold, int64_t num_refinement_steps,
                                              float* ref_corr_points, float* src_corr_points, float* corr_scores, int32_t* corr_patch,
                                              int32_t* num_corr, float* estimated_transform, int64_t transform_ld, float* patch_transforms,
                                              int32_t* patch_inliers, int32_t* best_patch, void* workspace, size_t workspace_bytes,
                                              void* stream);

int geob200_weighted_procrustes(const float* src_points, const float* ref_points, const float* weights, int64_t batch,
                                int64_t n, float weight_thresh, float eps, float* transforms, void* stream);

size_t geob200_node_correspondences_batched_workspace_bytes(int64_t n_rows, int64_t n_products, int64_t k);
int geob200_node_correspondences_batched(const float* ref_nodes, const float* src_nodes, const float* ref_knn_points,
                                         const float* src_knn_points, const uint8_t* ref_masks, const uint8_t* src_masks,
                                         const uint8_t* ref_knn_masks, const uint8_t* src_knn_masks, int64_t n_pairs, const int64_t* cloud_nodes,
                                         int64_t k, const float* transforms, float pos_radius, int64_t* corr_indices, float* corr_overlaps,
                                         int32_t* count, void* workspace, size_t workspace_bytes, void* stream);

int geob200_evaluate_counts(const int64_t* gt_node_corr_indices, const float* gt_node_corr_overlaps, int64_t n_gt, const int32_t* n_gt_dev,
                            float acceptance_overlap, const int64_t* ref_node_corr_indices, const int64_t* src_node_corr_indices,
                            int64_t n_node_corr, const int32_t* n_node_corr_dev, const float* ref_corr_points, const float* src_corr_points,
                            int64_t n_corr, const int32_t* n_corr_dev, float acceptance_radius, const float* gt_transform,
                            const float* est_transform, const float* src_points, int64_t n_src_points, int mode, float rmse_threshold,
                            float rre_threshold, float rte_threshold, float* metrics, void* stream);
int geob200_evaluate_batched(const int64_t* gt_node_corr_indices, const float* gt_node_corr_overlaps, const int32_t* n_gt_dev,
                             float acceptance_overlap, const int64_t* ref_node_corr_indices, const int64_t* src_node_corr_indices,
                             int64_t n_node_corr, const int32_t* n_node_corr_dev, const float* ref_corr_points, const float* src_corr_points,
                             int64_t n_corr, const int32_t* n_corr_dev, float acceptance_radius, const float* gt_transforms,
                             const float* est_transforms, int64_t transform_ld, const float* points, int64_t n_pairs, const int64_t* cloud_nodes,
                             const int64_t* cloud_points, int mode, float rmse_threshold, float rre_threshold, float rte_threshold,
                             float* metrics, int64_t metrics_ld, void* stream);

size_t geob200_coarse_matching_loss_batched_workspace_bytes(int64_t n_rows, int64_t n_products);
int geob200_coarse_matching_loss_batched(const float* ref_feats, const float* src_feats, int64_t channels, int64_t n_pairs,
                                         const int64_t* cloud_nodes, const int64_t* gt_node_corr_indices, const float* gt_node_corr_overlaps,
                                         const int32_t* gt_count, float positive_margin, float negative_margin, float positive_optimal,
                                         float negative_optimal, float log_scale, float positive_overlap, float* out, int64_t out_ld,
                                         void* workspace, size_t workspace_bytes, void* stream);
size_t geob200_fine_matching_loss_batched_workspace_bytes(int64_t n_pairs, int64_t n_patches);
int geob200_fine_matching_loss_batched(const float* ref_knn_points, const float* src_knn_points, const uint8_t* ref_knn_masks,
                                       const uint8_t* src_knn_masks, const float* matching_scores, const float* transforms, int64_t n_pairs,
                                       int64_t n_patches, int64_t k, const int32_t* patch_count, double positive_radius,
                                       const float* loss_weights, float* out, int64_t out_ld, void* workspace, size_t workspace_bytes,
                                       void* stream);

size_t geob200_coarse_matching_loss_backward_batched_workspace_bytes(int64_t n_rows, int64_t n_products, int64_t n_pairs);
int geob200_coarse_matching_loss_backward_batched(const float* ref_feats, const float* src_feats, int64_t channels, int64_t n_pairs,
                                                  const int64_t* cloud_nodes, const int64_t* gt_node_corr_indices,
                                                  const float* gt_node_corr_overlaps, const int32_t* gt_count, float positive_margin,
                                                  float negative_margin, float positive_optimal, float negative_optimal, float log_scale,
                                                  float positive_overlap, const float* grad_rows, int64_t grad_ld, const float* loss_weights,
                                                  float* grad_ref_feats, float* grad_src_feats, void* workspace, size_t workspace_bytes,
                                                  void* stream);
size_t geob200_fine_matching_loss_backward_batched_workspace_bytes(int64_t n_pairs, int64_t n_patches);
int geob200_fine_matching_loss_backward_batched(const float* ref_knn_points, const float* src_knn_points, const uint8_t* ref_knn_masks,
                                                const uint8_t* src_knn_masks, const float* transforms, int64_t n_pairs, int64_t n_patches,
                                                int64_t k, const int32_t* patch_count, double positive_radius, const float* grad_rows,
                                                int64_t grad_ld, const float* loss_weights, float* grad_scores, void* workspace,
                                                size_t workspace_bytes, void* stream);

size_t geob200_ransac_correspondences_batched_workspace_bytes(int64_t n_pairs, int64_t num_iterations);
int geob200_ransac_correspondences_batched(const float* ref_corr_points, const float* src_corr_points, int64_t n_pairs, int64_t capacity,
                                           const int32_t* num_corr, float distance_threshold, int64_t ransac_n, int64_t num_iterations,
                                           uint64_t seed, int64_t pair_base, float* transforms, float* fitness, float* inlier_rmse,
                                           int32_t* inlier_count,
                                           int32_t* best_iteration, float* hyp_transforms, int32_t* hyp_inliers, float* hyp_rmse,
                                           int32_t* hyp_samples, void* workspace, size_t workspace_bytes, void* stream);

size_t geob200_correspondence_metrics_batched_workspace_bytes(int64_t n_pairs, int64_t capacity);
int geob200_correspondence_metrics_batched(const float* ref_corr_points, const float* src_corr_points, int64_t n_pairs, int64_t capacity,
                                           const int32_t* num_corr, const float* transforms, int64_t transform_ld, float positive_radius,
                                           float* out, int64_t out_ld, void* workspace, size_t workspace_bytes, void* stream);

size_t geob200_feature_nn_batched_workspace_bytes(int64_t n_pairs, int64_t cap_query, int64_t cap_support);
int geob200_feature_nn_batched(const float* query, const float* support, int64_t n_pairs, int64_t cap_query, int64_t cap_support,
                               int64_t channels, const int32_t* n_query, const int32_t* n_support, int64_t* query_index,
                               double* query_dist, int64_t* support_index, double* support_dist, void* workspace, size_t workspace_bytes,
                               void* stream);
int geob200_feature_corr_indices(const int64_t* ref_nn, const double* ref_dist, const int64_t* src_nn, const double* src_dist,
                                 int64_t n_ref, int64_t n_src, int32_t mode, int64_t* ref_corr, int64_t* src_corr, float* feat_dist,
                                 int32_t* count, void* stream);
size_t geob200_ransac_features_batched_workspace_bytes(int64_t n_pairs, int64_t cap_src, int64_t cap_ref, int64_t num_iterations,
                                                       int64_t val_iterations);
int geob200_ransac_features_batched(const float* src_points, const float* ref_points, const float* src_feats, const float* ref_feats,
                                    int64_t n_pairs, int64_t cap_src, int64_t cap_ref, int64_t channels, const int32_t* n_src,
                                    const int32_t* n_ref, float distance_threshold, int64_t ransac_n, int64_t num_iterations,
                                    int64_t val_iterations, uint64_t seed, int64_t pair_base, float* transforms, float* fitness,
                                    float* inlier_rmse, int32_t* inlier_count, int32_t* best_iteration, int32_t* num_validated,
                                    int64_t* rec_matches, int32_t* rec_samples, int32_t* rec_pass, int32_t* rec_val_ids,
                                    float* rec_transforms, int32_t* rec_inliers, float* rec_rmse, void* workspace, size_t workspace_bytes,
                                    void* stream);

int geob200_corr_order_batched(const float* scores, int64_t n_pairs, int64_t capacity, const int32_t* num_corr, int64_t kmax, int32_t* order,
                               void* stream);
int geob200_corr_select_batched(const float* ref_corr_points, const float* src_corr_points, const float* corr_scores, int64_t n_pairs,
                                int64_t capacity, const int32_t* num_corr, const int32_t* order, int64_t kmax, int64_t k,
                                float* ref_out, float* src_out, float* scores_out, int32_t* count_out, void* stream);
size_t geob200_sparse_correspondence_eval_batched_workspace_bytes(int64_t n_pairs, int64_t m_cap, int64_t n_cap);
int geob200_sparse_correspondence_eval_batched(const int64_t* ref_node_corr_indices, const int64_t* src_node_corr_indices, int64_t pred_cap,
                                               const int32_t* pred_count, const int64_t* gt_node_corr_indices, int64_t gt_cap,
                                               const int32_t* gt_count, int64_t n_pairs, int64_t m_cap, int64_t n_cap, double* out,
                                               void* workspace, size_t workspace_bytes, void* stream);
int geob200_registration_error_batched(const float* gt_transforms, int64_t gt_ld, const float* est_transforms, int64_t est_ld,
                                       const float* covariances, const int32_t* has_covariance, int64_t n_pairs, int mode,
                                       double threshold0, double threshold1, double* out, void* stream);
int geob200_weighted_procrustes_counts(const float* src_points, const float* ref_points, const float* weights, int64_t batch,
                                       int64_t capacity, const int32_t* counts, float weight_thresh, float eps, float* transforms,
                                       void* stream);

int geob200_linear_profile_enable(int on);
int geob200_set_split_k(int on);
int geob200_set_linear_persistent(int on);
int64_t geob200_linear_profile_read(int64_t capacity, int64_t* shapes, float* ms);

#define GEOB200_MAX_STAGES 6
typedef struct { const float* weight; const float* bias; int64_t c_in, c_out; const float* weight_img; } geob200_linear_t;
typedef struct { const float* gamma; const float* beta; } geob200_norm_t;
typedef struct { const float* weights; const float* weights_t; const float* bias; const float* kernel_points;
                 int64_t c_in, c_out; float sigma; const float* weights_img; } geob200_kpconv_t;
typedef struct {
    int32_t has_unary1, has_shortcut, strided, reserved;
    int64_t c_in;
    geob200_linear_t unary1; geob200_norm_t norm1;
    geob200_kpconv_t conv;   geob200_norm_t norm_conv;
    geob200_linear_t unary2; geob200_norm_t norm2;
    geob200_linear_t shortcut; geob200_norm_t norm_sc;
} geob200_resblock_t;
typedef struct {
    int32_t num_stages, finest_decoder, groups, init_dim;
    geob200_kpconv_t conv1; geob200_norm_t norm1;
    geob200_resblock_t blocks[1 + 3 * (GEOB200_MAX_STAGES - 1)];
    geob200_linear_t decoders[GEOB200_MAX_STAGES];
    geob200_norm_t decoder_norms[GEOB200_MAX_STAGES];
} geob200_backbone_t;
size_t geob200_backbone_workspace_bytes(const geob200_backbone_t* net, const int64_t* level_rows);
int geob200_backbone_forward_batched(const geob200_backbone_t* net, const float* feats, const float* const* points,
                                     const int64_t* level_rows, const int64_t* const* neighbors, const int64_t* neighbor_width,
                                     const int64_t* const* subsampling, const int64_t* subsampling_width,
                                     const int64_t* const* upsampling, const int64_t* upsampling_width, float* const* out_feats,
                                     void* gn_workspace, size_t gn_workspace_bytes, void* workspace, size_t workspace_bytes, void* stream,
                                     int64_t n_pairs, const int64_t* const* cloud_rows_h, const int32_t* const* sub_cloud_max);

typedef struct {
    int32_t is_self, reserved;
    const float* w_qkv; const float* b_qkv; const float* w_q; const float* b_q; const float* w_kv; const float* b_kv;
    const float* wp_t; const float* bp;
    geob200_linear_t att_linear; geob200_norm_t att_norm;
    geob200_linear_t expand; geob200_linear_t squeeze; geob200_norm_t out_norm;
    const float* w_qkv_img; const float* w_q_img; const float* w_kv_img;
} geob200_tlayer_t;
size_t geob200_transformer_batched_workspace_bytes(int64_t n_pairs, const int64_t* cloud_rows_h, int64_t channels, int64_t heads,
                                                   int64_t num_layers);
int geob200_transformer_forward_batched(const geob200_tlayer_t* layers, int64_t num_layers, int64_t channels, int64_t heads,
                                        const float* x, int64_t n_pairs, const int64_t* cloud_rows_h, const float* const* embeddings_h,
                                        float* out, void* workspace, size_t workspace_bytes, void* stream);

size_t geob200_superpoint_targets_batched_workspace_bytes(int64_t n_gt_rows);
int geob200_superpoint_targets_batched(const int64_t* gt_indices, const float* gt_overlaps, const int32_t* gt_count, int64_t n_pairs,
                                       const int64_t* cloud_nodes, float overlap_threshold, int64_t num_targets, uint64_t seed,
                                       uint64_t iteration, int64_t pair_base, int64_t* corr_indices, float* corr_scores, int32_t* num_out,
                                       void* workspace, size_t workspace_bytes, void* stream);

int geob200_nonfinite_check(const float* const* ptrs, const int64_t* numels, int64_t n_tensors, int64_t max_numel, float* found_inf,
                            void* stream);

int geob200_batch_loss_weights(const float* loss_rows, int64_t ld_rows, int64_t n_pairs, float* weights, float* mean_row, float* n_valid,
                               float* found_inf, void* stream);

#define GEOB200_AUGMENT_3DMATCH 0
#define GEOB200_AUGMENT_KITTI 1
#define GEOB200_AUGMENT_TAG_BASE 0xA6000000u

size_t geob200_augment_pairs_batched_workspace_bytes(int64_t n_rows);
int geob200_augment_pairs_batched(const float* points, const int64_t* lengths_h, int64_t n_pairs, const float* transforms, int mode,
                                  int64_t point_limit, double noise, double rotation_factor, double min_scale, double max_scale,
                                  double shift, uint64_t seed, uint64_t iteration, int64_t pair_base, float* out_points, int32_t* origin,
                                  float* out_transforms, double* record, void* workspace, size_t workspace_bytes, void* stream);

size_t geob200_modelnet_pairs_batched_workspace_bytes(int64_t n_rows);
int geob200_modelnet_pairs_batched(const float* shapes, const int64_t* lengths_h, int64_t n_pairs, int64_t num_points, double keep_ratio,
                                   double rotation_magnitude, double translation_magnitude, double noise_magnitude, uint64_t seed,
                                   uint64_t iteration, int64_t pair_base, float* out_points, int32_t* origin, float* out_transforms,
                                   double* record, void* workspace, size_t workspace_bytes, void* stream);

size_t geob200_modelnet_benchmark_pairs_batched_workspace_bytes(int64_t n_pairs, int64_t num_points);
int geob200_modelnet_benchmark_pairs_batched(const float* shapes, const int64_t* lengths_h, const int64_t* indices_h, int64_t n_pairs,
                                             int64_t num_points, double keep_ratio, double rotation_magnitude, double translation_magnitude,
                                             double noise_magnitude, float* out_points, int32_t* origin, float* out_transforms,
                                             void* workspace, size_t workspace_bytes, void* stream);

int geob200_rotated_pairs_batched(const void* points, int points_fp64, const int64_t* lengths_h, const int64_t* indices_h, int64_t n_pairs,
                                  const double* transforms, float* out_points, float* out_transforms, double* rotations, void* stream);


size_t geob200_modelnet_raw_points_batched_workspace_bytes(int64_t n_shapes);
int geob200_modelnet_raw_points_batched(const float* shapes, const int64_t* lengths_h, int64_t n_shapes, float* out_points,
                                        void* workspace, size_t workspace_bytes, void* stream);

#define GEOB200_RPMNET_MAX_PAIRS 32
#define GEOB200_RPMNET_COLUMNS 8
#define GEOB200_RPMNET_GT_DET 1
#define GEOB200_RPMNET_EST_DET 2
size_t geob200_rpmnet_metrics_batched_workspace_bytes(int64_t n_pairs, int64_t cap_query, int64_t cap_raw);
int geob200_rpmnet_metrics_batched(const float* raw, const int64_t* raw_lengths_h, const float* ref, const int64_t* ref_lengths_h,
                                   const float* src, const int64_t* src_lengths_h, int64_t n_pairs, const float* gt_transforms,
                                   const float* est_transforms, double* out, void* workspace, size_t workspace_bytes, void* stream);

#ifdef __cplusplus
}
#endif
#endif
```

Baseline: 427.7.

## Batch all stage radius searches into one stacked multi-grid launch sequence

Replaces the per-search radius search calls in data precomputation (neighbors, subsampling and upsampling for every stage) with one stacked call. That call builds the spatial grids for all point sets together and runs every query over a single flattened grid of blocks. The query loop now merges the nine neighbouring cell ranges into one flat index space, so each warp processes full 32-wide chunks instead of looping per row. The cell scan also handles four elements per thread. The aim is to cut launch count, host round-trips and warp underutilisation, at the cost of more complex descriptors and a binary search per query to find its cloud.

```diff
diff --git a/geotransformer_b200/_lib.py b/geotransformer_b200/_lib.py
--- a/geotransformer_b200/_lib.py
+++ b/geotransformer_b200/_lib.py
@@ -25,6 +25,8 @@
 _sig('geob200_grid_subsample', c_int, P, I64, P, I64, F, P, P, P, SZ, P)
 _sig('geob200_radius_search_workspace_bytes', SZ, I64, I64, I64)
 _sig('geob200_radius_search', c_int, P, I64, P, I64, P, P, I64, F, I64, P, P, P, P, SZ, P)
+_sig('geob200_radius_search_stack_workspace_bytes', SZ, P, I64, I64, P, P, P, I64)
+_sig('geob200_radius_search_stack', c_int, P, P, P, I64, I64, P, P, P, P, P, P, I64, P, SZ, P)
 
 _sig('geob200_neighbor_histogram', c_int, P, I64, I64, I64, I64, P, P)
 _sig('geob200_neighbor_histogram_batched', c_int, P, P, P, I64, I64, I64, I64, P, P, P, P)
diff --git a/geotransformer_b200/csrc/collate.cu b/geotransformer_b200/csrc/collate.cu
--- a/geotransformer_b200/csrc/collate.cu
+++ b/geotransformer_b200/csrc/collate.cu
@@ -39,19 +39,21 @@
 }
 
 
-__global__ void __launch_bounds__(1024) seg_exclusive_scan_kernel(const int* __restrict__ in, int* __restrict__ out,
-                                                                  const CloudSeg* __restrict__ segs,
-                                                                  int* __restrict__ total) {
+__device__ __forceinline__ int block_exclusive_scan(const int* __restrict__ in, int* __restrict__ out, int len) {
     __shared__ int warp_tot[32];
     __shared__ int carry_s;
-    const CloudSeg sg = segs[blockIdx.x];
     const int lane = threadIdx.x & 31, warp = threadIdx.x >> 5;
     if (threadIdx.x == 0) carry_s = 0;
     __syncthreads();
-    for (int base = 0; base < sg.len; base += 1024) {
-        int i = base + threadIdx.x;
-        int v = (i < sg.len) ? in[sg.start + i] : 0;
-        int x = v;
+    for (int base = 0; base < len; base += 4 * 1024) {
+        const int i0 = base + 4 * threadIdx.x;
+        int v[4], s = 0;
+#pragma unroll
+        for (int k = 0; k < 4; ++k) {
+            v[k] = (i0 + k < len) ? in[i0 + k] : 0;
+            s += v[k];
+        }
+        int x = s;
 #pragma unroll
         for (int o = 1; o < 32; o <<= 1) {
             int y = __shfl_up_sync(0xffffffffu, x, o);
@@ -69,14 +71,26 @@
             warp_tot[lane] = w;
         }
         __syncthreads();
-        int carry = carry_s;
-        int excl = carry + (warp > 0 ? warp_tot[warp - 1] : 0) + (x - v);
-        if (i < sg.len) out[sg.start + i] = excl;
+        const int carry = carry_s;
+        int excl = carry + (warp > 0 ? warp_tot[warp - 1] : 0) + (x - s);
+#pragma unroll
+        for (int k = 0; k < 4; ++k) {
+            if (i0 + k < len) out[i0 + k] = excl;
+            excl += v[k];
+        }
         __syncthreads();
         if (threadIdx.x == 1023) carry_s = carry + warp_tot[31];
         __syncthreads();
     }
-    if (threadIdx.x == 0 && total != nullptr) total[blockIdx.x] = carry_s;
+    return carry_s;
+}
+
+__global__ void __launch_bounds__(1024) seg_exclusive_scan_kernel(const int* __restrict__ in, int* __restrict__ out,
+                                                                  const CloudSeg* __restrict__ segs,
+                                                                  int* __restrict__ total) {
+    const CloudSeg sg = segs[blockIdx.x];
+    const int t = block_exclusive_scan(in + sg.start, out + sg.start, sg.len);
+    if (threadIdx.x == 0 && total != nullptr) total[blockIdx.x] = t;
 }
 
 
@@ -289,6 +303,10 @@
 }
 
 
+#define RS_MAX_SETS 8
+#define RS_MAX_GRIDS 8
+#define RS_MAX_SEARCHES 16
+
 struct RsCloud {
     float ox, oy, oz;
     float cell;
@@ -296,14 +314,49 @@
     int cell_base;
 };
 
-__global__ void __launch_bounds__(1024) rs_bounds_kernel(const float* __restrict__ pts, const CloudSeg* __restrict__ segs,
-                                                         float radius, RsCloud* __restrict__ out, CloudSeg* __restrict__ cell_segs,
-                                                         int* __restrict__ max_count) {
-    if (blockIdx.x == 0 && threadIdx.x == 0) *max_count = 0;
-    const CloudSeg sg = segs[blockIdx.x];
+struct RsGridDesc {
+    const float* pts;
+    int set;
+    float radius;
+    int cell_off;
+    int pt_off;
+};
+
+struct RsGrids {
+    RsGridDesc g[RS_MAX_GRIDS];
+    int n;
+    int batch;
+    int* max_count[RS_MAX_SEARCHES];
+    int n_search;
+};
+
+struct RsSearchDesc {
+    const float* q_pts;
+    int q_set, grid;
+    int rows;
+    int block_begin;
+    int width;
+    float radius;
+    long long sentinel;
+    long long* out;
+    int* counts;
+    int* max_count;
+};
+
+struct RsSearches {
+    RsSearchDesc s[RS_MAX_SEARCHES];
+    int n;
+    int batch;
+};
+
+__global__ void __launch_bounds__(1024) rs_bounds_kernel(RsGrids gd, const CloudSeg* __restrict__ segs, RsCloud* __restrict__ out) {
+    const int b = blockIdx.x, gi = blockIdx.y;
+    if (b == 0 && gi == 0 && threadIdx.x < gd.n_search) *gd.max_count[threadIdx.x] = 0;
+    const RsGridDesc g = gd.g[gi];
+    const CloudSeg sg = segs[g.set * gd.batch + b];
     float mn[3] = {INFINITY, INFINITY, INFINITY}, mx[3] = {-INFINITY, -INFINITY, -INFINITY};
     for (int i = threadIdx.x; i < sg.len; i += blockDim.x) {
-        const float* p = pts + 3ll * (sg.start + i);
+        const float* p = g.pts + 3ll * (sg.start + i);
 #pragma unroll
         for (int a = 0; a < 3; ++a) { mn[a] = fminf(mn[a], p[a]); mx[a] = fmaxf(mx[a], p[a]); }
     }
@@ -326,7 +379,7 @@
         RsCloud c;
         c.ox = smn[0][0]; c.oy = smn[1][0]; c.oz = smn[2][0];
         const long long budget = 2ll * sg.len + 1024;
-        float cell = radius * 1.001f;
+        float cell = g.radius * 1.001f;
         long long cx, cy, cz;
         while (true) {
             cx = (long long)floorf((smx[0][0] - c.ox) / cell) + 1;
@@ -336,10 +389,8 @@
             cell *= 1.25f;
         }
         c.cell = cell; c.cx = (int)cx; c.cy = (int)cy; c.cz = (int)cz;
-        c.cell_base = 2 * sg.start + 1025 * blockIdx.x;
-        out[blockIdx.x] = c;
-        cell_segs[blockIdx.x].start = c.cell_base;
-        cell_segs[blockIdx.x].len = c.cx * c.cy * c.cz + 1;
+        c.cell_base = g.cell_off + 2 * sg.start + 1025 * b;
+        out[gi * gd.batch + b] = c;
     }
 }
 
@@ -349,41 +400,37 @@
     return (iz * c.cy + iy) * c.cx + ix;
 }
 
-__global__ void rs_count_kernel(const float* __restrict__ pts, const CloudSeg* __restrict__ segs,
-                                const RsCloud* __restrict__ clouds, int* __restrict__ cell_cnt, int* __restrict__ pt_cell) {
-    const CloudSeg sg = segs[blockIdx.y];
+__global__ void rs_count_kernel(RsGrids gd, const CloudSeg* __restrict__ segs, const RsCloud* __restrict__ clouds,
+                                int* __restrict__ cell_cnt, int* __restrict__ pt_cell) {
+    const RsGridDesc g = gd.g[blockIdx.z];
+    const CloudSeg sg = segs[g.set * gd.batch + blockIdx.y];
     const int i = blockIdx.x * blockDim.x + threadIdx.x;
     if (i >= sg.len) return;
-    const RsCloud c = clouds[blockIdx.y];
-    const float* p = pts + 3ll * (sg.start + i);
+    const RsCloud c = clouds[blockIdx.z * gd.batch + blockIdx.y];
+    const float* p = g.pts + 3ll * (sg.start + i);
     const int cell = rs_cell_of(c, p[0], p[1], p[2]);
-    pt_cell[sg.start + i] = cell;
+    pt_cell[g.pt_off + sg.start + i] = cell;
     atomicAdd(&cell_cnt[c.cell_base + cell], 1);
 }
 
-__global__ void rs_scatter_kernel(const float* __restrict__ pts, const CloudSeg* __restrict__ segs,
-                                  const RsCloud* __restrict__ clouds, const int* __restrict__ cell_start,
-                                  int* __restrict__ cell_cursor, const int* __restrict__ pt_cell,
+__global__ void __launch_bounds__(1024) rs_cell_scan_kernel(int batch, const RsCloud* __restrict__ clouds,
+                                                            const int* __restrict__ cell_cnt, int* __restrict__ cell_start) {
+    const RsCloud c = clouds[blockIdx.y * batch + blockIdx.x];
+    block_exclusive_scan(cell_cnt + c.cell_base, cell_start + c.cell_base, c.cx * c.cy * c.cz + 1);
+}
+
+__global__ void rs_scatter_kernel(RsGrids gd, const CloudSeg* __restrict__ segs, const RsCloud* __restrict__ clouds,
+                                  const int* __restrict__ cell_start, int* __restrict__ cell_cursor, const int* __restrict__ pt_cell,
                                   float4* __restrict__ sorted) {
-    const CloudSeg sg = segs[blockIdx.y];
+    const RsGridDesc g = gd.g[blockIdx.z];
+    const CloudSeg sg = segs[g.set * gd.batch + blockIdx.y];
     const int i = blockIdx.x * blockDim.x + threadIdx.x;
     if (i >= sg.len) return;
-    const RsCloud c = clouds[blockIdx.y];
-    const int cell = pt_cell[sg.start + i];
+    const RsCloud c = clouds[blockIdx.z * gd.batch + blockIdx.y];
+    const int cell = pt_cell[g.pt_off + sg.start + i];
     const int pos = atomicAdd(&cell_cursor[c.cell_base + cell], 1);
-    const float* p = pts + 3ll * (sg.start + i);
-    sorted[sg.start + cell_start[c.cell_base + cell] + pos] = make_float4(p[0], p[1], p[2], __int_as_float(i));
-}
-
-struct RsSegs {
-    int start, len;
-};
-__global__ void rs_cellsegs_kernel(const RsCloud* __restrict__ clouds, int nb, CloudSeg* __restrict__ cell_segs) {
-    int b = blockIdx.x * blockDim.x + threadIdx.x;
-    if (b >= nb) return;
-    const RsCloud c = clouds[b];
-    cell_segs[b].start = c.cell_base;
-    cell_segs[b].len = c.cx * c.cy * c.cz + 1;
+    const float* p = g.pts + 3ll * (sg.start + i);
+    sorted[g.pt_off + sg.start + cell_start[c.cell_base + cell] + pos] = make_float4(p[0], p[1], p[2], __int_as_float(i));
 }
 
 template <int KPL>
@@ -434,76 +481,112 @@
     for (int e = 32 * KPL + lane; e < width; e += 32) orow[e] = sentinel;
 }
 
+__device__ __forceinline__ int rs_cloud_of(const CloudSeg* __restrict__ segs, int batch, int row) {
+    int lo = 0, hi = batch - 1;
+    while (lo < hi) {
+        const int mid = (lo + hi + 1) >> 1;
+        if (segs[mid].start <= row) lo = mid;
+        else hi = mid - 1;
+    }
+    return lo;
+}
+
+struct RsTables {
+    const CloudSeg* segs;
+    const RsCloud* clouds;
+    const int* cell_start;
+    const float4* sorted;
+    int batch;
+};
+
 template <int CAP>
-__device__ __forceinline__ void rs_query_body(unsigned long long* buf, int lane, int b, int qi,
-                                              const float* __restrict__ q_pts, const CloudSeg* __restrict__ q_segs,
-                                              const CloudSeg* __restrict__ s_segs, const RsCloud* __restrict__ clouds,
-                                              const int* __restrict__ cell_start, const float4* __restrict__ sorted,
-                                              float radius, int width, long long sentinel, long long* __restrict__ out,
-                                              int* __restrict__ counts, int* __restrict__ max_count,
-                                              int* __restrict__ overflow_list, int* __restrict__ overflow_n) {
-    const CloudSeg qs = q_segs[b];
-    const CloudSeg ss = s_segs[b];
-    const RsCloud c = clouds[b];
-    const long long row = (long long)qs.start + qi;
-    const float qx = q_pts[3 * row], qy = q_pts[3 * row + 1], qz = q_pts[3 * row + 2];
-    const float r2 = __fmul_rn(radius, radius);
+__device__ __forceinline__ void rs_query_body(unsigned long long* buf, int lane, int si, const RsSearchDesc& sd, const RsGridDesc& g,
+                                              int row, const RsTables& tb, int2* __restrict__ overflow_list,
+                                              int* __restrict__ overflow_n) {
+    const int b = rs_cloud_of(tb.segs + sd.q_set * tb.batch, tb.batch, row);
+    const CloudSeg ss = tb.segs[g.set * tb.batch + b];
+    const RsCloud c = tb.clouds[sd.grid * tb.batch + b];
+    const float qx = sd.q_pts[3ll * row], qy = sd.q_pts[3ll * row + 1], qz = sd.q_pts[3ll * row + 2];
+    const float r2 = __fmul_rn(sd.radius, sd.radius);
     const float lim = 2.0e6f;
     const int ix = (int)fminf(fmaxf(floorf((qx - c.ox) / c.cell), -lim), lim);
     const int iy = (int)fminf(fmaxf(floorf((qy - c.oy) / c.cell), -lim), lim);
     const int iz = (int)fminf(fmaxf(floorf((qz - c.oz) / c.cell), -lim), lim);
+    const int x0 = max(ix - 1, 0), x1 = min(ix + 1, c.cx - 1);
+    int beg = 0, len = 0;
+    if (lane < 9) {
+        const int z = iz + lane / 3 - 1, y = iy + lane % 3 - 1;
+        if (x0 <= x1 && z >= 0 && z < c.cz && y >= 0 && y < c.cy) {
+            const int rowcell = c.cell_base + (z * c.cy + y) * c.cx;
+            beg = tb.cell_start[rowcell + x0];
+            len = tb.cell_start[rowcell + x1 + 1] - beg;
+        }
+    }
+    int incl = len;
+#pragma unroll
+    for (int o = 1; o < 16; o <<= 1) {
+        const int y = __shfl_up_sync(0xffffffffu, incl, o);
+        if (lane >= o) incl += y;
+    }
+    const int total = __shfl_sync(0xffffffffu, incl, 8);
+    int first[9], shift[9];
+#pragma unroll
+    for (int j = 0; j < 9; ++j) {
+        first[j] = __shfl_sync(0xffffffffu, incl - len, j);
+        shift[j] = __shfl_sync(0xffffffffu, beg - (incl - len), j);
+    }
+    const float4* sp = tb.sorted + g.pt_off + ss.start;
     int count = 0;
-    const int x0 = max(ix - 1, 0), x1 = min(ix + 1, c.cx - 1);
-    if (x0 <= x1) {
-        for (int dz = -1; dz <= 1; ++dz) {
-            const int z = iz + dz;
-            if (z < 0 || z >= c.cz) continue;
-            for (int dy = -1; dy <= 1; ++dy) {
-                const int y = iy + dy;
-                if (y < 0 || y >= c.cy) continue;
-                const int rowcell = c.cell_base + (z * c.cy + y) * c.cx;
-                const int beg = cell_start[rowcell + x0], end = cell_start[rowcell + x1 + 1];
-                const int end_pad = beg + ((end - beg + 31) / 32) * 32;
-                for (int k = beg + lane; k < end_pad; k += 32) {
-                    bool hit = false;
-                    unsigned long long kv = 0;
-                    if (k < end) {
-                        const float4 s = sorted[ss.start + k];
-                        const float ex = __fsub_rn(qx, s.x), ey = __fsub_rn(qy, s.y), ez = __fsub_rn(qz, s.z);
-                        float d = __fmul_rn(ex, ex);
-                        d = __fadd_rn(d, __fmul_rn(ey, ey));
-                        d = __fadd_rn(d, __fmul_rn(ez, ez));
-                        hit = d < r2;
-                        kv = ((unsigned long long)__float_as_uint(d) << 32) | (unsigned)__float_as_int(s.w);
-                    }
-                    const unsigned msk = __ballot_sync(0xffffffffu, hit);
-                    if (hit) {
-                        const int pos = count + __popc(msk & ((1u << lane) - 1u));
-                        if (pos < CAP) buf[pos] = kv;
-                    }
-                    count += __popc(msk);
-                }
-            }
-        }
+    for (int t0 = 0; t0 < total; t0 += 32) {
+        const int t = t0 + lane;
+        bool hit = false;
+        unsigned long long kv = 0;
+        if (t < total) {
+            int sh = shift[0];
+#pragma unroll
+            for (int j = 1; j < 9; ++j) sh = (t >= first[j]) ? shift[j] : sh;
+            const float4 s = sp[t + sh];
+            const float ex = __fsub_rn(qx, s.x), ey = __fsub_rn(qy, s.y), ez = __fsub_rn(qz, s.z);
+            float d = __fmul_rn(ex, ex);
+            d = __fadd_rn(d, __fmul_rn(ey, ey));
+            d = __fadd_rn(d, __fmul_rn(ez, ez));
+            hit = d < r2;
+            kv = ((unsigned long long)__float_as_uint(d) << 32) | (unsigned)__float_as_int(s.w);
+        }
+        const unsigned msk = __ballot_sync(0xffffffffu, hit);
+        if (hit) {
+            const int pos = count + __popc(msk & ((1u << lane) - 1u));
+            if (pos < CAP) buf[pos] = kv;
+        }
+        count += __popc(msk);
     }
     if (count > CAP) {
         if (lane == 0) {
-            if (overflow_list != nullptr) overflow_list[atomicAdd(overflow_n, 1)] = (int)row;
-            else atomicExch(max_count, -1 << 30);
+            if (overflow_list != nullptr) overflow_list[atomicAdd(overflow_n, 1)] = make_int2(si, row);
+            else atomicExch(sd.max_count, -1 << 30);
         }
         return;
     }
     if (lane == 0) {
-        if (counts != nullptr) counts[row] = count;
-        atomicMax(max_count, count);
-    }
-    if (out == nullptr || width <= 0) return;
+        if (sd.counts != nullptr) sd.counts[row] = count;
+        atomicMax(sd.max_count, count);
+    }
+    const int width = sd.width;
+    if (sd.out == nullptr || width <= 0) return;
     __syncwarp();
-    long long* orow = out + row * (long long)width;
-    if (count <= 32) rs_sort_and_store<1>(buf, count, lane, orow, width, ss.start, sentinel);
-    else if (count <= 64) rs_sort_and_store<2>(buf, count, lane, orow, width, ss.start, sentinel);
-    else if (count <= 128) rs_sort_and_store<4>(buf, count, lane, orow, width, ss.start, sentinel);
-    else if (count <= 256) rs_sort_and_store<8>(buf, count, lane, orow, width, ss.start, sentinel);
+    long long* orow = sd.out + (long long)row * width;
+    if (count <= 32) {
+        if (lane < count) {
+            const unsigned long long mine = buf[lane];
+            int rank = 0;
+            for (int j = 0; j < count; ++j) rank += buf[j] < mine ? 1 : 0;
+            if (rank < width) orow[rank] = (long long)(unsigned)(mine & 0xFFFFFFFFull) + ss.start;
+        }
+        for (int e = count + lane; e < width; e += 32) orow[e] = sd.sentinel;
+    }
+    else if (count <= 64) rs_sort_and_store<2>(buf, count, lane, orow, width, ss.start, sd.sentinel);
+    else if (count <= 128) rs_sort_and_store<4>(buf, count, lane, orow, width, ss.start, sd.sentinel);
+    else if (count <= 256) rs_sort_and_store<8>(buf, count, lane, orow, width, ss.start, sd.sentinel);
     else {
         int n2 = 1;
         while (n2 < count) n2 <<= 1;
@@ -523,44 +606,186 @@
             }
         }
         for (int k = lane; k < width; k += 32)
-            orow[k] = (k < count) ? (long long)(unsigned)(buf[k] & 0xFFFFFFFFull) + ss.start : sentinel;
-    }
+            orow[k] = (k < count) ? (long long)(unsigned)(buf[k] & 0xFFFFFFFFull) + ss.start : sd.sentinel;
+    }
+}
+
+template <int CAP, int WARPS>
+__global__ void __launch_bounds__(WARPS * 32) rs_query_kernel(RsSearches srch, RsGrids gd, RsTables tb, int2* __restrict__ overflow_list,
+                                                              int* __restrict__ overflow_n) {
+    extern __shared__ unsigned long long smem_keys[];
+    int si = 0;
+    while (si + 1 < srch.n && (int)blockIdx.x >= srch.s[si + 1].block_begin) ++si;
+    const RsSearchDesc& sd = srch.s[si];
+    const int lane = threadIdx.x & 31, warp = threadIdx.x >> 5;
+    const int row = ((int)blockIdx.x - sd.block_begin) * WARPS + warp;
+    if (row >= sd.rows) return;
+    rs_query_body<CAP>(smem_keys + (size_t)warp * CAP, lane, si, sd, gd.g[sd.grid], row, tb, overflow_list, overflow_n);
 }
 
 template <int CAP>
-__global__ void rs_query_kernel(const float* __restrict__ q_pts, const CloudSeg* __restrict__ q_segs,
-                                const CloudSeg* __restrict__ s_segs, const RsCloud* __restrict__ clouds,
-                                const int* __restrict__ cell_start, const float4* __restrict__ sorted, float radius,
-                                int width, long long sentinel, long long* __restrict__ out, int* __restrict__ counts,
-                                int* __restrict__ max_count, int* __restrict__ overflow_list, int* __restrict__ overflow_n) {
-    extern __shared__ unsigned long long smem_keys[];
-    const int warps_per_block = blockDim.x >> 5;
-    const int lane = threadIdx.x & 31, warp = threadIdx.x >> 5;
-    const int b = blockIdx.y;
-    const int qi = blockIdx.x * warps_per_block + warp;
-    if (qi >= q_segs[b].len) return;
-    rs_query_body<CAP>(smem_keys + (size_t)warp * CAP, lane, b, qi, q_pts, q_segs, s_segs, clouds, cell_start, sorted,
-                       radius, width, sentinel, out, counts, max_count, overflow_list, overflow_n);
-}
-
-template <int CAP>
-__global__ void rs_redo_kernel(const float* __restrict__ q_pts, const CloudSeg* __restrict__ q_segs,
-                               const CloudSeg* __restrict__ s_segs, const RsCloud* __restrict__ clouds,
-                               const int* __restrict__ cell_start, const float4* __restrict__ sorted, float radius,
-                               int width, long long sentinel, long long* __restrict__ out, int* __restrict__ counts,
-                               int* __restrict__ max_count, const int* __restrict__ redo_list,
-                               const int* __restrict__ redo_n, int nbatch) {
+__global__ void rs_redo_kernel(RsSearches srch, RsGrids gd, RsTables tb, const int2* __restrict__ redo_list,
+                               const int* __restrict__ redo_n) {
     extern __shared__ unsigned long long smem_keys[];
     const int n = *redo_n;
     for (int w = blockIdx.x; w < n; w += gridDim.x) {
-        const int row = redo_list[w];
-        int b = 0;
-        while (b + 1 < nbatch && row >= q_segs[b + 1].start) ++b;
-        rs_query_body<CAP>(smem_keys, threadIdx.x, b, row - q_segs[b].start, q_pts, q_segs, s_segs, clouds, cell_start,
-                           sorted, radius, width, sentinel, out, counts, max_count, nullptr, nullptr);
+        const int2 e = redo_list[w];
+        const RsSearchDesc& sd = srch.s[e.x];
+        rs_query_body<CAP>(smem_keys, threadIdx.x, e.x, sd, gd.g[sd.grid], e.y, tb, nullptr, nullptr);
         __syncwarp();
     }
 }
+
+struct RsLayout {
+    int n_grids;
+    int grid_of[RS_MAX_SEARCHES];
+    int grid_set[RS_MAX_GRIDS];
+    float grid_radius[RS_MAX_GRIDS];
+    long long cell_off[RS_MAX_GRIDS], pt_off[RS_MAX_GRIDS];
+    long long cells, pts, queries;
+};
+
+static int rs_layout(const int64_t* set_rows, int64_t num_sets, int64_t batch, int64_t num_searches, const int64_t* q_set,
+                     const int64_t* s_set, const float* radius, RsLayout* L) {
+    GEOB_REQUIRE(num_sets >= 1 && num_sets <= RS_MAX_SETS, "radius_search: 1..%d point sets", RS_MAX_SETS);
+    GEOB_REQUIRE(num_searches >= 1 && num_searches <= RS_MAX_SEARCHES, "radius_search: 1..%d searches per call", RS_MAX_SEARCHES);
+    GEOB_REQUIRE(batch > 0, "radius_search: empty input");
+    L->n_grids = 0;
+    L->cells = L->pts = L->queries = 0;
+    for (int s = 0; s < (int)num_searches; ++s) {
+        GEOB_REQUIRE(q_set[s] >= 0 && q_set[s] < num_sets && s_set[s] >= 0 && s_set[s] < num_sets, "radius_search: bad set index");
+        GEOB_REQUIRE(radius[s] > 0.f, "radius_search: radius must be positive");
+        int g = 0;
+        while (g < L->n_grids && !(L->grid_set[g] == (int)s_set[s] && L->grid_radius[g] == radius[s])) ++g;
+        if (g == L->n_grids) {
+            GEOB_REQUIRE(g < RS_MAX_GRIDS, "radius_search: more than %d distinct (support, radius) grids", RS_MAX_GRIDS);
+            L->grid_set[g] = (int)s_set[s];
+            L->grid_radius[g] = radius[s];
+            L->cell_off[g] = L->cells;
+            L->pt_off[g] = L->pts;
+            L->cells += 2 * set_rows[s_set[s]] + 1025 * batch + 64;
+            L->pts += set_rows[s_set[s]];
+            ++L->n_grids;
+        }
+        L->grid_of[s] = g;
+        L->queries += set_rows[q_set[s]];
+    }
+    GEOB_REQUIRE(L->cells < (1ll << 31) && L->pts < (1ll << 31), "radius_search: too many points");
+    return 0;
+}
+
+static size_t rs_workspace_bytes(const RsLayout& L, int64_t num_sets, int64_t batch) {
+    size_t bytes = 0;
+    bytes += align_up(sizeof(CloudSeg) * num_sets * batch, 256) + align_up(sizeof(RsCloud) * L.n_grids * batch, 256);
+    bytes += align_up(4 * (2 * L.cells + 64), 256);
+    bytes += align_up(4 * L.cells, 256);
+    bytes += align_up(4 * L.pts, 256);
+    bytes += align_up(16 * L.pts, 256);
+    bytes += align_up(8 * L.queries, 256);
+    return bytes + 4096;
+}
+
+static int rs_run(const float* const* set_points, const int64_t* set_rows, const int64_t* set_lengths_h, int64_t num_sets, int64_t batch,
+                  const int64_t* q_set, const int64_t* s_set, const float* radius, const int64_t* width, int64_t* const* out,
+                  int32_t* const* counts, int32_t* const* max_count, int64_t num_searches, void* workspace, size_t workspace_bytes,
+                  cudaStream_t st) {
+    RsLayout L;
+    if (int e = rs_layout(set_rows, num_sets, batch, num_searches, q_set, s_set, radius, &L)) return e;
+    GEOB_REQUIRE(workspace_bytes >= rs_workspace_bytes(L, num_sets, batch), "radius_search: workspace too small");
+    bool support[RS_MAX_SETS] = {};
+    for (int s = 0; s < (int)num_searches; ++s) {
+        support[s_set[s]] = true;
+        GEOB_REQUIRE(max_count[s] != nullptr, "radius_search: max_count output is required");
+        GEOB_REQUIRE(set_rows[q_set[s]] > 0 && set_rows[s_set[s]] > 0, "radius_search: empty input");
+    }
+    CloudSeg tmp[RS_MAX_SETS * 64];
+    CloudSeg* h = tmp;
+    CloudSeg* heap = nullptr;
+    if (num_sets * batch > RS_MAX_SETS * 64) { heap = (CloudSeg*)malloc(sizeof(CloudSeg) * num_sets * batch); h = heap; }
+    int max_len[RS_MAX_SETS] = {};
+    for (int k = 0; k < (int)num_sets; ++k) {
+        GEOB_REQUIRE(set_rows[k] < (1ll << 30), "radius_search: too many points");
+        int64_t acc = 0;
+        for (int64_t b = 0; b < batch; ++b) {
+            const int64_t n = set_lengths_h[k * batch + b];
+            if (n < 0 || (support[k] && n == 0)) {
+                free(heap);
+                GEOB_REQUIRE(false, "radius_search: cloud %lld has no support points", (long long)b);
+            }
+            h[k * batch + b].start = (int)acc;
+            h[k * batch + b].len = (int)n;
+            acc += n;
+            max_len[k] = n > max_len[k] ? (int)n : max_len[k];
+        }
+        if (acc != set_rows[k]) {
+            free(heap);
+            GEOB_REQUIRE(false, "radius_search: lengths do not sum to the row counts");
+        }
+    }
+    Arena ar(workspace, workspace_bytes);
+    CloudSeg* segs = ar.take<CloudSeg>(num_sets * batch);
+    RsCloud* clouds = ar.take<RsCloud>(L.n_grids * batch);
+    int* zero_block = ar.take<int>(2 * L.cells + 64);
+    int* cell_cnt = zero_block;
+    int* cell_cursor = zero_block + L.cells;
+    int* overflow_n = zero_block + 2 * L.cells;
+    int* cell_start = ar.take<int>(L.cells);
+    int* pt_cell = ar.take<int>(L.pts);
+    float4* sorted = ar.take<float4>(L.pts);
+    int2* overflow_list = ar.take<int2>(L.queries);
+    if (!ar.ok()) { free(heap); GEOB_REQUIRE(false, "radius_search: workspace accounting error"); }
+    cudaError_t e = cudaMemcpyAsync(segs, h, sizeof(CloudSeg) * num_sets * batch, cudaMemcpyHostToDevice, st);
+    if (heap) { cudaStreamSynchronize(st); free(heap); }
+    GEOB_REQUIRE(e == cudaSuccess, "radius_search: %s", cudaGetErrorString(e));
+    GEOB_CHECK_CUDA(cudaMemsetAsync(zero_block, 0, 4 * (2 * L.cells + 64), st));
+
+    RsGrids gd{};
+    gd.n = L.n_grids;
+    gd.batch = (int)batch;
+    gd.n_search = (int)num_searches;
+    int max_s = 0;
+    for (int g = 0; g < L.n_grids; ++g) {
+        gd.g[g] = RsGridDesc{set_points[L.grid_set[g]], L.grid_set[g], L.grid_radius[g], (int)L.cell_off[g], (int)L.pt_off[g]};
+        max_s = max_len[L.grid_set[g]] > max_s ? max_len[L.grid_set[g]] : max_s;
+    }
+    constexpr int CAP = 256, WARPS = 4;
+    RsSearches srch{};
+    srch.n = (int)num_searches;
+    srch.batch = (int)batch;
+    long long blocks = 0;
+    for (int s = 0; s < (int)num_searches; ++s) {
+        gd.max_count[s] = max_count[s];
+        RsSearchDesc& d = srch.s[s];
+        d.q_pts = set_points[q_set[s]];
+        d.q_set = (int)q_set[s];
+        d.grid = L.grid_of[s];
+        d.rows = (int)set_rows[q_set[s]];
+        d.block_begin = (int)blocks;
+        d.width = (int)width[s];
+        d.radius = radius[s];
+        d.sentinel = (long long)set_rows[s_set[s]];
+        d.out = (long long*)out[s];
+        d.counts = counts != nullptr ? counts[s] : nullptr;
+        d.max_count = max_count[s];
+        blocks += (d.rows + WARPS - 1) / WARPS;
+    }
+    GEOB_REQUIRE(blocks < (1ll << 31), "radius_search: too many queries");
+    const RsTables tb{segs, clouds, cell_start, sorted, (int)batch};
+    const dim3 cgrid((unsigned)batch, (unsigned)L.n_grids);
+    const dim3 sgrid((max_s + 255) / 256, (unsigned)batch, (unsigned)L.n_grids);
+    rs_bounds_kernel<<<cgrid, 1024, 0, st>>>(gd, segs, clouds);
+    rs_count_kernel<<<sgrid, 256, 0, st>>>(gd, segs, clouds, cell_cnt, pt_cell);
+    rs_cell_scan_kernel<<<cgrid, 1024, 0, st>>>((int)batch, clouds, cell_cnt, cell_start);
+    rs_scatter_kernel<<<sgrid, 256, 0, st>>>(gd, segs, clouds, cell_start, cell_cursor, pt_cell, sorted);
+    rs_query_kernel<CAP, WARPS><<<(unsigned)blocks, WARPS * 32, WARPS * CAP * 8, st>>>(srch, gd, tb, overflow_list, overflow_n);
+    constexpr int CAP2 = 16384;
+    if (ensure_max_smem((const void*)rs_redo_kernel<CAP2>)) return -1;
+    rs_redo_kernel<CAP2><<<num_sms(), 32, CAP2 * 8, st>>>(srch, gd, tb, overflow_list, overflow_n);
+    GEOB_CHECK_LAUNCH();
+    count_launches(6);
+    return 0;
+}
+
 
 __global__ void __launch_bounds__(256) neighbor_histogram_kernel(const long long* __restrict__ nbr, long long rows, int width,
                                                                  long long n_support, int hist_n, int* __restrict__ hist) {
@@ -716,77 +941,52 @@
 }
 
 size_t geob200_radius_search_workspace_bytes(int64_t n_query, int64_t n_support, int64_t batch) {
-    size_t ns = (size_t)n_support, nq = (size_t)n_query, b = (size_t)batch;
-    size_t cells = 2 * ns + 1025 * b + 64;
-    size_t bytes = 0;
-    bytes += align_up(sizeof(CloudSeg) * b, 256) * 3 + align_up(sizeof(RsCloud) * b, 256);
-    bytes += align_up(4 * cells, 256) * 3 + 1024;
-    bytes += align_up(4 * ns, 256);
-    bytes += align_up(16 * ns, 256);
-    bytes += align_up(4 * nq, 256);
-    bytes += 1024;
-    return bytes + 4096;
+    const int64_t rows[2] = {n_query, n_support}, q_set = 0, s_set = 1;
+    const float radius = 1.f;
+    RsLayout L;
+    if (rs_layout(rows, 2, batch, 1, &q_set, &s_set, &radius, &L)) return 0;
+    return rs_workspace_bytes(L, 2, batch);
 }
 
 int geob200_radius_search(const float* q_points, int64_t n_query, const float* s_points, int64_t n_support,
                           const int64_t* q_lengths_h, const int64_t* s_lengths_h, int64_t batch, float radius,
                           int64_t width, int64_t* out, int32_t* counts, int32_t* max_count, void* workspace,
                           size_t workspace_bytes, void* stream) {
-    cudaStream_t st = (cudaStream_t)stream;
     GEOB_REQUIRE(batch > 0 && n_query > 0 && n_support > 0, "radius_search: empty input");
     GEOB_REQUIRE(radius > 0.f, "radius_search: radius must be positive");
     GEOB_REQUIRE(max_count != nullptr, "radius_search: max_count output is required");
     GEOB_REQUIRE(n_query < (1ll << 30) && n_support < (1ll << 30), "radius_search: too many points");
-    GEOB_REQUIRE(workspace_bytes >= geob200_radius_search_workspace_bytes(n_query, n_support, batch), "radius_search: workspace too small");
-    for (int64_t b = 0; b < batch; ++b)
-        GEOB_REQUIRE(q_lengths_h[b] >= 0 && s_lengths_h[b] > 0, "radius_search: cloud %lld has no support points", (long long)b);
-    Arena ar(workspace, workspace_bytes);
-    const size_t ns = (size_t)n_support;
-    const size_t cells = 2 * ns + 1025 * (size_t)batch + 64;
-    CloudSeg* q_segs = ar.take<CloudSeg>(batch);
-    CloudSeg* s_segs = ar.take<CloudSeg>(batch);
-    CloudSeg* cell_segs = ar.take<CloudSeg>(batch);
-    RsCloud* clouds = ar.take<RsCloud>(batch);
-    int* zero_block = ar.take<int>(2 * cells + 64);
-    int* cell_cnt = zero_block;
-    int* cell_cursor = zero_block + cells;
-    int* overflow_n = zero_block + 2 * cells;
-    int* cell_start = ar.take<int>(cells);
-    int* pt_cell = ar.take<int>(ns);
-    float4* sorted = ar.take<float4>(ns);
-    int* overflow_list = ar.take<int>((size_t)n_query);
-    GEOB_REQUIRE(ar.ok(), "radius_search: workspace accounting error");
-
-    int64_t tq = 0, ts = 0;
-    int max_q = 0, max_s = 0;
-    if (upload_segs(q_lengths_h, batch, q_segs, &tq, &max_q, st)) return -1;
-    if (upload_segs(s_lengths_h, batch, s_segs, &ts, &max_s, st)) return -1;
-    GEOB_REQUIRE(tq == n_query && ts == n_support, "radius_search: lengths do not sum to the row counts");
-
-    GEOB_CHECK_CUDA(cudaMemsetAsync(zero_block, 0, 4 * (2 * cells + 64), st));
-
-    const dim3 sgrid((max_s + 255) / 256, (unsigned)batch);
-    rs_bounds_kernel<<<(unsigned)batch, 1024, 0, st>>>(s_points, s_segs, radius, clouds, cell_segs, max_count);
-    rs_count_kernel<<<sgrid, 256, 0, st>>>(s_points, s_segs, clouds, cell_cnt, pt_cell);
-    seg_exclusive_scan_kernel<<<(unsigned)batch, 1024, 0, st>>>(cell_cnt, cell_start, cell_segs, nullptr);
-    rs_scatter_kernel<<<sgrid, 256, 0, st>>>(s_points, s_segs, clouds, cell_start, cell_cursor, pt_cell, sorted);
-    if (max_q > 0) {
-        constexpr int CAP = 256, WARPS = 4;
-        const dim3 qgrid((max_q + WARPS - 1) / WARPS, (unsigned)batch);
-        rs_query_kernel<CAP><<<qgrid, WARPS * 32, WARPS * CAP * 8, st>>>(
-            q_points, q_segs, s_segs, clouds, cell_start, sorted, radius, (int)width, (long long)n_support,
-            (long long*)out, counts, max_count, overflow_list, overflow_n);
-        constexpr int CAP2 = 16384;
-        if (ensure_max_smem((const void*)rs_redo_kernel<CAP2>)) return -1;
-        rs_redo_kernel<CAP2><<<num_sms(), 32, CAP2 * 8, st>>>(
-            q_points, q_segs, s_segs, clouds, cell_start, sorted, radius, (int)width, (long long)n_support,
-            (long long*)out, counts, max_count, overflow_list, overflow_n, (int)batch);
-        count_launches(2);
-    }
-    GEOB_CHECK_LAUNCH();
-    count_launches(4);
-    return 0;
-}
+    const float* pts[2] = {q_points, s_points};
+    const int64_t rows[2] = {n_query, n_support}, q_set = 0, s_set = 1;
+    int64_t* lengths = (int64_t*)malloc(sizeof(int64_t) * 2 * batch);
+    GEOB_REQUIRE(lengths != nullptr, "radius_search: out of host memory");
+    memcpy(lengths, q_lengths_h, sizeof(int64_t) * batch);
+    memcpy(lengths + batch, s_lengths_h, sizeof(int64_t) * batch);
+    const int rc = rs_run(pts, rows, lengths, 2, batch, &q_set, &s_set, &radius, &width, &out, &counts, &max_count, 1, workspace,
+                          workspace_bytes, (cudaStream_t)stream);
+    free(lengths);
+    return rc;
+}
+
+size_t geob200_radius_search_stack_workspace_bytes(const int64_t* set_rows, int64_t num_sets, int64_t batch, const int64_t* q_set,
+                                                   const int64_t* s_set, const float* radius, int64_t num_searches) {
+    RsLayout L;
+    if (rs_layout(set_rows, num_sets, batch, num_searches, q_set, s_set, radius, &L)) return 0;
+    return rs_workspace_bytes(L, num_sets, batch);
+}
+
+int geob200_radius_search_stack(const float* const* set_points, const int64_t* set_rows, const int64_t* set_lengths_h, int64_t num_sets,
+                                int64_t batch, const int64_t* q_set, const int64_t* s_set, const float* radius, const int64_t* width,
+                                int64_t* const* out, int32_t* max_count, int64_t num_searches, void* workspace, size_t workspace_bytes,
+                                void* stream) {
+    GEOB_REQUIRE(num_searches >= 1 && num_searches <= RS_MAX_SEARCHES, "radius_search: 1..%d searches per call", RS_MAX_SEARCHES);
+    GEOB_REQUIRE(max_count != nullptr, "radius_search: max_count output is required");
+    int32_t* mc[RS_MAX_SEARCHES];
+    for (int s = 0; s < (int)num_searches; ++s) mc[s] = max_count + s;
+    return rs_run(set_points, set_rows, set_lengths_h, num_sets, batch, q_set, s_set, radius, width, out, nullptr, mc, num_searches,
+                  workspace, workspace_bytes, (cudaStream_t)stream);
+}
+
 
 int geob200_neighbor_histogram(const int64_t* neighbors, int64_t n_rows, int64_t width, int64_t n_support, int64_t hist_n,
                                int32_t* hist, void* stream) {
diff --git a/geotransformer_b200/ext.py b/geotransformer_b200/ext.py
--- a/geotransformer_b200/ext.py
+++ b/geotransformer_b200/ext.py
@@ -1,4 +1,7 @@
 
+import ctypes
+
+import numpy as np
 import torch
 
 from . import _lib as L
@@ -76,6 +79,33 @@
     return out.cpu() if was_cpu else out
 
 
+def radius_neighbors_stack(points, lengths_h, searches):
+    for i, p in enumerate(points):
+        if p.dtype != torch.float32 or not p.is_contiguous():
+            raise RuntimeError(f'points[{i}] must be a contiguous float tensor')
+    points = [p if p.is_cuda else p.cuda() for p in points]
+    lib = L.lib()
+    dev = points[0].device
+    k, b, n = len(points), int(lengths_h[0].shape[0]), len(searches)
+    rows = np.array([p.shape[0] for p in points], dtype=np.int64)
+    lens = np.concatenate([np.asarray(l, dtype=np.int64) for l in lengths_h])
+    q_set = np.array([s[0] for s in searches], dtype=np.int64)
+    s_set = np.array([s[1] for s in searches], dtype=np.int64)
+    radius = np.array([s[2] for s in searches], dtype=np.float32)
+    width = np.array([s[3] for s in searches], dtype=np.int64)
+    tables = [torch.empty((points[q].shape[0], int(w)), dtype=torch.int64, device=dev) for q, w in zip(q_set, width)]
+    max_count = torch.empty((n,), dtype=torch.int32, device=dev)
+    pts_p = (ctypes.c_void_p * k)(*[p.data_ptr() for p in points])
+    out_p = (ctypes.c_void_p * n)(*[L.ptr(t) for t in tables])
+    ws_bytes = lib.geob200_radius_search_stack_workspace_bytes(rows.ctypes.data, k, b, q_set.ctypes.data, s_set.ctypes.data,
+                                                               radius.ctypes.data, n)
+    ws = L.workspace(ws_bytes, dev)
+    L.check(lib.geob200_radius_search_stack(pts_p, rows.ctypes.data, lens.ctypes.data, k, b, q_set.ctypes.data, s_set.ctypes.data,
+                                            radius.ctypes.data, width.ctypes.data, out_p, max_count.data_ptr(), n, ws.data_ptr(),
+                                            ws.numel(), L.stream_ptr()), 'radius_neighbors')
+    return tables, max_count
+
+
 def radius_neighbors_deferred(q_points, s_points, q_lengths, s_lengths, radius, neighbor_limit):
     q_points, ql_h, _ = _prep(q_points, q_lengths, 'q_points', 'q_lengths')
     s_points, sl_h, _ = _prep(s_points, s_lengths, 's_points', 's_lengths')
diff --git a/geotransformer_b200/modules/ops/__init__.py b/geotransformer_b200/modules/ops/__init__.py
--- a/geotransformer_b200/modules/ops/__init__.py
+++ b/geotransformer_b200/modules/ops/__init__.py
@@ -13,8 +13,8 @@
     return _ext.radius_neighbors(q_points, s_points, q_lengths, s_lengths, radius, neighbor_limit=max(int(neighbor_limit), 0))
 
 
-def radius_search_deferred(q_points, s_points, q_lengths, s_lengths, radius, neighbor_limit):
-    return _ext.radius_neighbors_deferred(q_points, s_points, q_lengths, s_lengths, radius, int(neighbor_limit))
+def radius_search_stack(points, lengths, searches):
+    return _ext.radius_neighbors_stack(points, lengths, [(q, s, r, int(w)) for q, s, r, w in searches])
 
 
 def point_to_node_partition(points, nodes, point_limit, return_count=False):
diff --git a/geotransformer_b200/utils/data.py b/geotransformer_b200/utils/data.py
--- a/geotransformer_b200/utils/data.py
+++ b/geotransformer_b200/utils/data.py
@@ -3,7 +3,7 @@
 import numpy as np
 import torch
 
-from ..modules.ops import grid_subsample, radius_search_deferred
+from ..modules.ops import grid_subsample, radius_search_stack
 
 
 def precompute_data_stack_mode(points, lengths, num_stages, voxel_size, radius, neighbor_limits):
@@ -18,19 +18,18 @@
         lengths_list.append(lengths_h.to(points.device))
         voxel_size *= 2
 
-    pending = []
+    kinds, searches = [], []
     for i in range(num_stages):
-        cur_points, cur_lengths = points_list[i], lengths_host[i]
-        pending.append(('n', radius_search_deferred(cur_points, cur_points, cur_lengths, cur_lengths, radius, neighbor_limits[i])))
+        kinds.append('n')
+        searches.append((i, i, radius, neighbor_limits[i]))
         if i < num_stages - 1:
-            sub_points, sub_lengths = points_list[i + 1], lengths_host[i + 1]
-            pending.append(('s', radius_search_deferred(sub_points, cur_points, sub_lengths, cur_lengths, radius, neighbor_limits[i])))
-            pending.append(('u', radius_search_deferred(cur_points, sub_points, cur_lengths, sub_lengths, radius * 2,
-                                                        neighbor_limits[i + 1])))
+            kinds += ['s', 'u']
+            searches += [(i + 1, i, radius, neighbor_limits[i]), (i, i + 1, radius * 2, neighbor_limits[i + 1])]
         radius *= 2
-    counts = torch.stack([p[1][1] for p in pending]).cpu().flatten().tolist()
+    tables, max_counts = radius_search_stack(points_list, lengths_host, searches)
+    counts = max_counts.cpu().tolist()
     neighbors_list, subsampling_list, upsampling_list = [], [], []
-    for (kind, (table, _)), mc in zip(pending, counts):
+    for kind, table, mc in zip(kinds, tables, counts):
         if mc < 0:
             raise RuntimeError('radius_search: more than 16384 neighbours for one query')
         if mc < table.shape[1]:
diff --git a/include/geob200.h b/include/geob200.h
--- a/include/geob200.h
+++ b/include/geob200.h
@@ -21,6 +21,13 @@
                           const int64_t* q_lengths_h, const int64_t* s_lengths_h, int64_t batch, float radius,
                           int64_t width, int64_t* out, int32_t* counts, int32_t* max_count, void* workspace,
                           size_t workspace_bytes, void* stream);
+
+size_t geob200_radius_search_stack_workspace_bytes(const int64_t* set_rows, int64_t num_sets, int64_t batch, const int64_t* q_set,
+                                                   const int64_t* s_set, const float* radius, int64_t num_searches);
+int geob200_radius_search_stack(const float* const* set_points, const int64_t* set_rows, const int64_t* set_lengths_h, int64_t num_sets,
+                                int64_t batch, const int64_t* q_set, const int64_t* s_set, const float* radius, const int64_t* width,
+                                int64_t* const* out, int32_t* max_count, int64_t num_searches, void* workspace, size_t workspace_bytes,
+                                void* stream);
 
 int geob200_neighbor_histogram(const int64_t* neighbors, int64_t n_rows, int64_t width, int64_t n_support, int64_t hist_n,
                                int32_t* hist, void* stream);
```

Result: no change. 428.6 (median of 6 runs) (+0.2%).
